# adammoss/nnest

Hardware: AMD Instinct MI355X
Metric: live-point evals/sec (flow-transform + loglike) + log-Z error, x_dim=50 (higher is better)
Workload: dtype f32

## Files before the change

### nnest_amd/csrc/mh_common.h

```cpp
#pragma once
#include "flow_tile.h"
#include "../../include/nnest_hip.h"

namespace nnest {

#ifdef NNEST_STAMP
#define STAMP(v) do { __builtin_amdgcn_sched_barrier(0); v = __builtin_amdgcn_s_memtime(); __builtin_amdgcn_s_waitcnt(0xC07F); __builtin_amdgcn_sched_barrier(0); } while (0)
#else
#define STAMP(v) do { } while (0)
#endif

enum { MH_FORM_AUTO = 0, MH_FORM_IMAGE = 1, MH_FORM_REG = 2, MH_FORM_TEAM = 3, MH_FORM_QUAD = 4, MH_FORM_QUAD1 = 5, MH_FORM_SOLO = 6 };
enum { NNEST_MH_ALL_MOVED = 1 << 30 };
enum { NNEST_MH_WINDOW_VOTES_ONLY = 1 << 28 };
__host__ __device__ inline int mh_flag_lag(int flags) { return (flags >> 8) & 15; }
__host__ __device__ inline int mh_flag_form(int flags) { return (flags >> 16) & 15; }
__host__ __device__ inline int mh_flag_warm(int flags) { return (flags >> 20) & 255; }

enum { MH_SYNC_SHARDS = 8, MH_SYNC_STRIDE = 8 , MH_SYNC_MAX_POLLS = 1 << 20 };
__host__ __device__ inline size_t mh_sync_counter_words(int steps) { return (size_t)(steps + 2) * MH_SYNC_SHARDS * MH_SYNC_STRIDE; }
__host__ __device__ inline size_t mh_sync_window_words(int steps) { return (size_t)((steps + 2) / 32 + 1) * MH_SYNC_SHARDS * MH_SYNC_STRIDE; }
__host__ __device__ inline size_t mh_sync_words(int steps) { return 2 * mh_sync_counter_words(steps) + mh_sync_window_words(steps); }

struct MhArgs {
    const float *img;
    FlowShape s;
    float *z;
    float *x;
    double *logl;
    double loglstar;
    float step_size;
    int steps;
    int C;
    int flags;
    LikeSpec like;
    const float *noise_dz;
    const float *noise_u;
    uint64_t seed;
    uint64_t walker_offset;
    float *hist_x;
    double *hist_logl;
    int *n_accept;
    int *n_call;
    float *scale_out;
    float *x0;
    const float *packed;
    unsigned long long *sync;
    int *sync_err;
};

struct SliceArgs {
    float *z, *x;
    double *logl;
    double loglstar;
    float width;
    int steps, C, max_out, max_shrink;
    LikeSpec like;
    uint64_t seed, walker_offset;
    const float *noise_dz;
    float *hist_x;
    float *x0;
    int *n_call, *n_move, *n_eval;
};

float *mh_first_x_buffer(size_t floats, hipStream_t st);
hipError_t launch_mh_all_moved(const MhArgs &a, hipStream_t st);
hipError_t launch_mh_zero_other_sync(const MhArgs &a, hipStream_t st);

template <int NT>
struct XoshiroNoise {
    Xoshiro128 rn, ru;
    unsigned valid_mask;
    __device__ __forceinline__ void init(uint64_t seed, uint64_t walker, int g, int D) {
        rn = xoshiro_seed(seed, walker, (uint32_t)g, NOISE_STREAM_DZ);
        ru = xoshiro_seed(seed, walker, 0xffffffffu, NOISE_STREAM_U);
        valid_mask = 0;
#pragma unroll
        for (int t = 0; t < NT; ++t)
#pragma unroll
            for (int j = 0; j < 8; ++j)
                if (32 * t + 8 * g + j < D) valid_mask |= 1u << (8 * t + j);
    }
    __device__ __forceinline__ bool relays() const { return false; }
    __device__ __forceinline__ int relayed_total() const { return 0; }
    __device__ __forceinline__ void relay_count(int, int) const {}
    __device__ __forceinline__ void next(float (&nz)[NT][8], float &u) {
#pragma unroll
        for (int t = 0; t < NT; ++t) {
            xoshiro_normal8(rn, nz[t]);
#pragma unroll
            for (int j = 0; j < 8; ++j)
                if (!((valid_mask >> (8 * t + j)) & 1u)) nz[t][j] = 0.f;
        }
        u = xoshiro_uniform(ru);
    }
};

__device__ __forceinline__ void mh_sync_post(unsigned long long *sync, int it, int wg, int accepted) {
    unsigned long long *w = sync + ((size_t)it * MH_SYNC_SHARDS + (wg & (MH_SYNC_SHARDS - 1))) * MH_SYNC_STRIDE;
    __hip_atomic_fetch_add(w, (1ull << 32) | (unsigned long long)(unsigned)accepted, __ATOMIC_RELAXED, __HIP_MEMORY_SCOPE_AGENT);
}
__device__ __forceinline__ unsigned long long mh_sync_read(const unsigned long long *sync, int it) {
    const unsigned long long *w = sync + (size_t)it * MH_SYNC_SHARDS * MH_SYNC_STRIDE;
    unsigned long long s = 0;
#pragma unroll
    for (int k = 0; k < MH_SYNC_SHARDS; ++k)
        s += __hip_atomic_load(w + k * MH_SYNC_STRIDE, __ATOMIC_RELAXED, __HIP_MEMORY_SCOPE_AGENT);
    return s;
}
__device__ __forceinline__ bool mh_sync_failed(const int *err) {
    return err && __hip_atomic_load(err, __ATOMIC_RELAXED, __HIP_MEMORY_SCOPE_AGENT) != 0;
}
__device__ __forceinline__ void mh_sync_fail(int *err, int which = 1) {
    if (err) __hip_atomic_store(err, which, __ATOMIC_RELAXED, __HIP_MEMORY_SCOPE_AGENT);
}
__device__ __forceinline__ int mh_sync_total(const unsigned long long *sync, int it, int nwg, unsigned long long first, int *err) {
    unsigned long long s = first;
    int polls = 0;
    while ((int)(s >> 32) != nwg) {
        if ((polls & 255) == 0 && mh_sync_failed(err)) break;
        if (++polls > MH_SYNC_MAX_POLLS) {
            mh_sync_fail(err);
            break;
        }
        __builtin_amdgcn_s_sleep(2);
        s = mh_sync_read(sync, it);
    }
    return (int)(s & 0xffffffffull);
}

__device__ __forceinline__ void mh_sync_publisher(unsigned long long *sync, int steps, int last_step, int nwg, int nwalkers, int lane, int *err) {
    const int g = lane >> 3, sh = lane & 7;
    unsigned long long *results = sync + mh_sync_counter_words(steps);
    unsigned long long *windows = sync + 2 * mh_sync_counter_words(steps);
    unsigned int wbits = 0;
    int t0 = 1, polls = 0;
    while (t0 <= last_step) {
        const int t = t0 + g;
        const bool live = t <= last_step;
        unsigned long long v = 0;
        if (live) v = __hip_atomic_load(sync + ((size_t)t * MH_SYNC_SHARDS + sh) * MH_SYNC_STRIDE, __ATOMIC_RELAXED, __HIP_MEMORY_SCOPE_AGENT);
        v += __shfl_xor(v, 1);
        v += __shfl_xor(v, 2);
        v += __shfl_xor(v, 4);
        const bool done = live && (int)(v >> 32) == nwg;
        const unsigned long long bal = __ballot(done);
        int ndone = 0;
        while (ndone < 8 && ((bal >> (8 * ndone)) & 1ull)) ++ndone;
        if (g < ndone)
            __hip_atomic_store(results + ((size_t)t * MH_SYNC_SHARDS + sh) * MH_SYNC_STRIDE, (1ull << 63) | (v & 0xffffffffull),
                               __ATOMIC_RELAXED, __HIP_MEMORY_SCOPE_AGENT);
        if (ndone > 0) {
            const unsigned long long up = __ballot(done && 2 * (int)(v & 0xffffffffull) > nwalkers);
            for (int j = 0; j < ndone; ++j) {
                const int s_ = t0 + j, wi = (s_ - 1) >> 5, bi = (s_ - 1) & 31;
                wbits |= (unsigned int)((up >> (8 * j)) & 1ull) << bi;
                if (bi == 31 || j == ndone - 1) {
                    if (lane < MH_SYNC_SHARDS)
                        __hip_atomic_store(windows + ((size_t)wi * MH_SYNC_SHARDS + lane) * MH_SYNC_STRIDE,
                                           ((unsigned long long)(unsigned int)s_ << 32) | wbits, __ATOMIC_RELAXED, __HIP_MEMORY_SCOPE_AGENT);
                    if (bi == 31) wbits = 0;
                }
            }
        }
        t0 += ndone;
        if (ndone == 0) {
            if (++polls > MH_SYNC_MAX_POLLS || ((polls & 255) == 0 && mh_sync_failed(err))) {
                if (polls > MH_SYNC_MAX_POLLS) mh_sync_fail(err, 2);
                for (int tt = t0; tt <= last_step; ++tt)
                    if (lane < MH_SYNC_SHARDS) {
                        __hip_atomic_store(results + ((size_t)tt * MH_SYNC_SHARDS + lane) * MH_SYNC_STRIDE, 1ull << 63, __ATOMIC_RELAXED,
                                           __HIP_MEMORY_SCOPE_AGENT);
                        __hip_atomic_store(windows + ((size_t)((tt - 1) >> 5) * MH_SYNC_SHARDS + lane) * MH_SYNC_STRIDE,
                                           (unsigned long long)(unsigned int)last_step << 32, __ATOMIC_RELAXED, __HIP_MEMORY_SCOPE_AGENT);
                    }
                return;
            }
            __builtin_amdgcn_s_sleep(1);
        }
    }
}
__device__ __forceinline__ unsigned long long mh_result_load(const unsigned long long *sync, int steps, int it, int wg) {
    const unsigned long long *r = sync + mh_sync_counter_words(steps) + ((size_t)it * MH_SYNC_SHARDS + (wg & (MH_SYNC_SHARDS - 1))) * MH_SYNC_STRIDE;
    return __hip_atomic_load(r, __ATOMIC_RELAXED, __HIP_MEMORY_SCOPE_AGENT);
}
__device__ __forceinline__ int mh_result_wait(const unsigned long long *sync, int steps, int it, int wg, unsigned long long first, int *err) {
    unsigned long long v = first;
    int polls = 0;
    while (!(v >> 63)) {
        if ((polls & 255) == 0 && mh_sync_failed(err)) break;
        if (++polls > MH_SYNC_MAX_POLLS) {
            mh_sync_fail(err, 3);
            break;
        }
        __builtin_amdgcn_s_sleep(1);
        v = mh_result_load(sync, steps, it, wg);
    }
    return (int)(v & 0xffffffffull);
}

__device__ __forceinline__ unsigned long long mh_window_load(const unsigned long long *sync, int steps, int it, int wg) {
    const unsigned long long *w = sync + 2 * mh_sync_counter_words(steps) + ((size_t)((it - 1) >> 5) * MH_SYNC_SHARDS + (wg & (MH_SYNC_SHARDS - 1))) * MH_SYNC_STRIDE;
    return __hip_atomic_load(w, __ATOMIC_RELAXED, __HIP_MEMORY_SCOPE_AGENT);
}
__device__ __forceinline__ bool mh_window_vote(const unsigned long long *sync, int steps, int it, int wg, unsigned long long first, int *err) {
    unsigned long long v = first;
    int polls = 0;
    while ((int)(v >> 32) < it) {
        if ((polls & 255) == 0 && mh_sync_failed(err)) break;
        if (++polls > MH_SYNC_MAX_POLLS) {
            mh_sync_fail(err, 4 | (it << 8) | ((wg & 1023) << 20));
            break;
        }
        __builtin_amdgcn_s_sleep(1);
        v = mh_window_load(sync, steps, it, wg);
    }
    return ((v >> ((it - 1) & 31)) & 1ull) != 0;
}

}
```

### nnest_amd/csrc/nnest_solo.hip

```cpp
#include <string.h>
#include <mutex>
#include "mh_common.h"
#include "nnest_internal.h"
#include "solo_loglike.h"
#include "solo_schedule.h"
#include "solo_tile.h"

namespace nnest {

#ifdef NNEST_STAMP
#define PSTAMP(v) do { __builtin_amdgcn_sched_barrier(0); v = __builtin_amdgcn_s_memtime(); __builtin_amdgcn_s_waitcnt(0xC07F); __builtin_amdgcn_sched_barrier(0); } while (0)
#define PSTAMP_DRAINED(v) do { __builtin_amdgcn_sched_barrier(0); __builtin_amdgcn_s_waitcnt(0x0070); v = __builtin_amdgcn_s_memtime(); __builtin_amdgcn_s_waitcnt(0xC07F); __builtin_amdgcn_sched_barrier(0); } while (0)
#ifndef NNEST_STAMP_STEPS
#undef STAMP
#define STAMP(v) do { } while (0)
#endif
#else
#define PSTAMP(v) do { } while (0)
#define PSTAMP_DRAINED(v) do { } while (0)
#endif

static constexpr int SOLO_ETAB = 1024;
__device__ double solo_etab_dev[SOLO_ETAB];
__global__ void solo_etab_kernel() {
    const int k = blockIdx.x * blockDim.x + threadIdx.x;
    if (k < SOLO_ETAB) solo_etab_dev[k] = exp(1.0 / (double)(1 + k));
}
hipError_t solo_prepare_device(int device, hipStream_t st) {
    static std::mutex mu;
    static bool done[64];
    std::lock_guard<std::mutex> g(mu);
    if (device < 0 || device >= 64) return hipErrorInvalidDevice;
    if (done[device]) return hipSuccess;
    hipLaunchKernelGGL(solo_etab_kernel, dim3(SOLO_ETAB / 256), dim3(256), 0, st);
    hipError_t e = hipGetLastError();
    if (e == hipSuccess) e = hipStreamSynchronize(st);
    done[device] = e == hipSuccess;
    return e;
}

template <int U>
__global__ void __launch_bounds__(192) solo_image_kernel(const float *__restrict__ packed, float *__restrict__ limg, int D, int net_params) {
    const int lane = threadIdx.x & 63, b = threadIdx.x >> 6;
    SoloNet<U> nb;
    solo_gather<U>(nb, packed + (size_t)(b * 2 + (lane >= 32 ? 1 : 0)) * net_params, D, (b + 1) & 1, b & 1, lane);
    solo4_store<U>(limg, b, nb, lane);
}
hipError_t launch_solo_image(const float *packed, float *limg, const FlowShape &s, hipStream_t st) {
    if (!s.has_solo_image()) return hipErrorInvalidConfiguration;
    switch (s.NT) {
        case 1: hipLaunchKernelGGL(solo_image_kernel<1>, dim3(1), dim3(192), 0, st, packed, limg, s.D, s.net_params); break;
        case 2: hipLaunchKernelGGL(solo_image_kernel<2>, dim3(1), dim3(192), 0, st, packed, limg, s.D, s.net_params); break;
        case 3: hipLaunchKernelGGL(solo_image_kernel<3>, dim3(1), dim3(192), 0, st, packed, limg, s.D, s.net_params); break;
        case 4: hipLaunchKernelGGL(solo_image_kernel<4>, dim3(1), dim3(192), 0, st, packed, limg, s.D, s.net_params); break;
    }
    return hipGetLastError();
}

template <int U, int WPG> constexpr bool solo_lds_weights() { return U >= 3 || WPG > 4; }
template <int U, int WPG> constexpr int solo_reg_blocks() { return !solo_lds_weights<U, WPG>() ? 3 : (WPG == 4 ? 1 : (U <= 2 && WPG == 8 ? 1 : 0)); }

template <int U>
static __device__ __forceinline__ void solo_pin(float (&v)[2][U]) {
#pragma unroll
    for (int c = 0; c < 2; ++c)
#pragma unroll
        for (int u = 0; u < U; ++u) asm volatile("" : "+v"(v[c][u]));
}

typedef float solo_f32x2 __attribute__((ext_vector_type(2)));
#pragma clang fp contract(off)
static __device__ __forceinline__ double solo_rosenbrock2_paired(const LikeSpec &lk, int D, int lane, const float (&xs)[2][2], float &ld_ride) {
    const int i0 = 4 * (lane & 15);
    const solo_f32x2 sc = {lk.scale, lk.scale};
    const solo_f32x2 P = sc * solo_f32x2{xs[0][0], xs[0][1]};
    const solo_f32x2 Q = sc * solo_f32x2{xs[1][0], xs[1][1]};
    const solo_f32x2 R = {P.y, solo_ror<15>(P.x)};
    const solo_f32x2 aP = P * P, aQ = Q * Q;
    const solo_f32x2 bP = Q - aP, bQ = R - aQ;
    const solo_f32x2 cP = bP * bP, cQ = bQ * bQ;
    const solo_f32x2 eP = 100.0f * cP, eQ = 100.0f * cQ;
    const solo_f32x2 fP = 1.0f - P, fQ = 1.0f - Q;
    const solo_f32x2 qP = fP * fP, qQ = fQ * fQ;
    const solo_f32x2 tP = eP + qP, tQ = eQ + qQ;
    float facc = 0.f;
    facc = facc + ((i0 + 1 < D) ? tP.x : 0.f);
    facc = facc + ((i0 + 2 < D) ? tQ.x : 0.f);
    facc = facc + ((i0 + 3 < D) ? tP.y : 0.f);
    facc = facc + ((i0 + 4 < D) ? tQ.y : 0.f);
    solo_logdet_total_and_row_sum(ld_ride, facc);
    double acc = -(double)facc;
    if (!(fabs(acc) <= 1.79769313486231570e308)) acc = -1e100;
    return acc;
}
#pragma clang fp contract(fast)

enum { MH_SOLO_LAG_INTERNAL = 8 };
template <int U, bool DBG, int LK, int WPG>
__global__ void __launch_bounds__(64 * (WPG + 2)) mh_kernel_solo(MhArgs a) {
    extern __shared__ __attribute__((aligned(16))) float wlds[];
    __shared__ __attribute__((aligned(16))) float nbuf[2][WPG][16][2 * U];
    __shared__ float ubuf[2][WPG];
    __shared__ __attribute__((aligned(16))) uint32_t rawbuf[4 * WPG * 8 * U];
    __shared__ int acc_lds[2][WPG];
    __shared__ float fsbuf[2];
    __shared__ float fs_exact;
    __shared__ float fs_cand[2];
    __shared__ int vote_sel;
    __shared__ double etab[SOLO_ETAB];
    __shared__ __attribute__((aligned(16))) float x0buf[WPG][16][2 * U];

    const int lane = threadIdx.x & 63, wave = __builtin_amdgcn_readfirstlane(threadIdx.x >> 6);
    const int tile = blockIdx.x;
    const int D = a.s.D, S = a.steps, C = a.C;
    const bool recorded = DBG && a.noise_dz;
    const bool dynamic = (a.flags & NNEST_MH_DYNAMIC_BATCH) != 0;
    const bool use_tab = S + 2 <= SOLO_ETAB;
    const bool exact_all = dynamic && mh_flag_lag(a.flags) == 0;
    const bool direct_votes = (a.flags & NNEST_MH_WINDOW_VOTES_ONLY) == 0;
    const int lag = exact_all ? MH_SOLO_LAG_INTERNAL : mh_flag_lag(a.flags);
    const int warm = solo_warm_steps(S, mh_flag_warm(a.flags), dynamic, exact_all);
    constexpr bool LDSW = solo_lds_weights<U, WPG>();
    constexpr int RB = solo_reg_blocks<U, WPG>();
    const int ntiles = (C + WPG - 1) / WPG;
    if (tile >= ntiles) {
        if (dynamic && wave == 0) mh_sync_publisher(a.sync, S, exact_all ? S : max(S - lag, warm), ntiles, C, lane, a.sync_err);
        else if (dynamic && (a.flags & (NNEST_MH_SYNC_ZERO_NEXT | NNEST_MH_SYNC_ZERO_PREV))) {
            const size_t W = (size_t)mh_sync_words(S) + 1;
            unsigned long long *other = (a.flags & NNEST_MH_SYNC_ZERO_NEXT) ? a.sync + W : a.sync - W;
            const int nthr = (int)blockDim.x - 64;
            for (size_t i = threadIdx.x - 64; i < W; i += nthr) other[i] = 0ull;
        }
        return;
    }
    unsigned long long p0 = 0, p1 = 0, p2 = 0, p3 = 0, p4 = 0, p5 = 0, p6 = 0, p7 = 0, p8 = 0;
    (void)p0; (void)p1; (void)p2; (void)p3; (void)p4; (void)p5; (void)p6; (void)p7; (void)p8;
    PSTAMP(p0);
    const float *limg = a.img + a.s.solo_image_offset();
    const int j = wave;
    const int pos = lane & 15;
    const bool translate_half = lane >= 32;
    const bool writer_lane = lane < 16;
    const int row = tile * WPG + j;
    const bool ok = row < C;
    SoloNet<U> net[RB > 0 ? RB : 1];
    float z[2][U];
    double logl = 0.0;
    if (wave < WPG) {
        if constexpr (LDSW) {
            if constexpr (RB == 1) solo_image_load<U>(net[0], limg + (size_t)1 * SOLO4_NF * 64, lane);
        } else {
#pragma unroll
            for (int b = 0; b < 3; ++b) solo_image_load<U>(net[b], limg + (size_t)b * SOLO4_NF * 64, lane);
        }
#pragma unroll
        for (int u = 0; u < U; ++u)
#pragma unroll
            for (int c = 0; c < 2; ++c) {
                const int d = 2 * U * pos + 2 * u + c;
                z[c][u] = (ok && d < D) ? a.z[(size_t)row * D + d] : 0.f;
            }
        logl = ok ? a.logl[row] : 0.0;
    }
    if constexpr (LDSW) solo_image_to_lds<64 * (WPG + 2)>(wlds, limg);
    PSTAMP(p1);
    if (dynamic && use_tab)
        for (int k = threadIdx.x; k < S + 2; k += blockDim.x) etab[k] = solo_etab_dev[k];
    PSTAMP(p2);
    __syncthreads();
    PSTAMP(p3);

    if (wave == WPG) {
        const int g = lane & 3, j = min(lane >> 2, WPG - 1);
        const bool gen = lane < 4 * WPG;
        Xoshiro128 rn = xoshiro_seed(a.seed, a.walker_offset + (uint64_t)(tile * WPG + j), (uint32_t)g, NOISE_STREAM_DZ);
        Xoshiro128 ru = xoshiro_seed(a.seed, a.walker_offset + (uint64_t)(tile * WPG + j), 0xffffffffu, NOISE_STREAM_U);
        constexpr int NQ = 8 * WPG * U;
        unsigned long long n0 = 0, n1 = 0, n2 = 0, n_gen = 0, n_all = 0;
        (void)n0; (void)n1; (void)n2; (void)n_gen; (void)n_all;
        auto draw = [&](int k) {
            if (k > S) return;
            STAMP(n0);
            if (!recorded) {
                if (gen) {
#pragma unroll
                    for (int t = 0; t < 2 * U; ++t) {
                        u32x4 r;
                        r.x = xoshiro_next(rn); r.y = xoshiro_next(rn); r.z = xoshiro_next(rn); r.w = xoshiro_next(rn);
                        *reinterpret_cast<u32x4 *>(&rawbuf[lane * 8 * U + 4 * t]) = r;
                    }
                    const float u = xoshiro_uniform(ru);
                    if (g == 0) ubuf[k & 1][j] = u;
                }
                float *nb = &nbuf[k & 1][0][0][0];
#pragma unroll
                for (int i = 0; i < (NQ + 63) / 64; ++i) {
                    const int q = lane + 64 * i;
                    if (NQ % 64 == 0 || q < NQ) {
                        const u32x4 r = *reinterpret_cast<const u32x4 *>(&rawbuf[4 * q]);
                        const int sl = q / (2 * U), qq = q % (2 * U);
                        const int d0 = 32 * (qq >> 1) + 8 * (sl & 3) + 4 * (qq & 1);
                        float o0, o1, o2, o3;
                        box_muller(r.x, r.y, o0, o1);
                        box_muller(r.z, r.w, o2, o3);
                        const f32x4 o = {d0 < D ? o0 : 0.f, d0 + 1 < D ? o1 : 0.f, d0 + 2 < D ? o2 : 0.f, d0 + 3 < D ? o3 : 0.f};
                        *reinterpret_cast<f32x4 *>(nb + (sl >> 2) * 32 * U + d0) = o;
                    }
                }
            }
            if (!dynamic && lane == 0) fsbuf[k & 1] = a.step_size;
            STAMP(n1);
#ifdef NNEST_STAMP
            n_gen += n1 - n0;
#endif
        };
        STAMP(n2);
        draw(0);
        PSTAMP(p4);
        solo_barrier();
        PSTAMP(p5);
        if (S >= 1) {
            draw(1);
            solo_barrier();
            draw(2);
            for (int k = 1; k <= warm; ++k) {
                solo_barrier();
                solo_barrier();
                draw(k + 2);
                solo_barrier();
            }
            for (int k = solo_first_lagged_fetch(warm); k <= S; ++k) {
                solo_barrier();
                draw(k + 1);
            }
        }
#ifdef NNEST_STAMP
        { unsigned long long n3 = 0; STAMP(n3); n_all = n3 - n2; }
#endif
#ifdef NNEST_STAMP
        PSTAMP(p8);
        if (a.scale_out && lane == 0 && tile == 0) {
            float *o = a.scale_out;
            o[4] = (float)n_gen; o[5] = (float)n_all;
            o[32] = (float)(p1 - p0); o[33] = (float)(p2 - p1); o[34] = (float)(p3 - p2); o[35] = (float)(p4 - p3); o[36] = (float)(p5 - p4);
            o[37] = (float)(p8 - p5); o[38] = (float)(p8 - p0);
        }
#endif
#ifndef NNEST_STAMP
        if (!dynamic && a.scale_out && lane == 0) {
            const int g0 = (tile * WPG + 15) >> 4;
            if (16 * g0 < (tile + 1) * WPG && 16 * g0 < C) a.scale_out[g0] = a.step_size;
        }
#endif
        return;
    }
    if (wave == WPG + 1) {
        if (!dynamic) return;
        double scale = (double)a.step_size;
        int accept = 0, reject = 0;
        const int last = S - lag;
        const unsigned long long *wbase = a.sync + 2 * mh_sync_counter_words(S) + (size_t)(tile & (MH_SYNC_SHARDS - 1)) * MH_SYNC_STRIDE;
#define SOLO_RELAY_ITERATION(k_, q_)                                                                                        \
        {                                                                                                                   \
            const int k = (k_), want = k - lag;                                                                             \
              \
              \
              \
              \
              \
            asm volatile("s_waitcnt vmcnt(2)" : "+v"(q_) : : "memory");                                                     \
            if (want > warm) {                                                                                              \
                const bool up = mh_window_vote(a.sync, S, want, tile, q_, a.sync_err);                                      \
                if (up) accept += 1; else reject += 1;                                                                      \
                if (accept > reject) scale *= use_tab ? etab[accept] : exp(1.0 / (1 + accept));                             \
                if (accept < reject) scale /= use_tab ? etab[reject] : exp(1.0 / (1 + reject));                             \
            }                                                                                                               \
                   \
             \
            if (lane == 0) {                                                                                                \
                const int *ac = acc_lds[k & 1];                                                                             \
                const bool mine = k - 2 > warm;                                 \
                int acs = 0;                                                                                                \
                _Pragma("unroll") for (int w_ = 0; w_ < WPG; ++w_) acs += ac[w_];                                           \
                mh_sync_post(a.sync, mine ? k - 2 : 0, tile, mine ? acs : 0);                                               \
            }                                                                                                               \
            const int ask = min(max(want + 2, 1), max(last, 1));         \
            const unsigned long long *wp = wbase + (size_t)((ask - 1) >> 5) * MH_SYNC_SHARDS * MH_SYNC_STRIDE;              \
            asm volatile("global_load_dwordx2 %0, %1, off sc1" : "=v"(q_) : "v"(wp) : "memory");                            \
              \
            if (lane == 0) fsbuf[k & 1] = (float)scale;                                                                     \
            solo_barrier();                                                                           \
        }
        unsigned long long qa = 0, qb = 0;
        const int k0 = solo_relay_first_iteration(warm);
        if (warm > 0) {
            auto E = [&](int n) { return use_tab ? etab[n] : exp(1.0 / (1 + n)); };
            auto next_scale = [&](int acc, int rej, double sc) {
                if (acc > rej) sc *= E(acc);
                if (acc < rej) sc /= E(rej);
                return sc;
            };
            if (lane == 0) {
                fsbuf[0] = (float)scale;
                fs_cand[0] = (float)next_scale(accept + 1, reject, scale);
                fs_cand[1] = (float)next_scale(accept, reject + 1, scale);
            }
            solo_barrier();
            if (lane == 0) fsbuf[1] = (float)scale;
            solo_barrier();
            for (int k = 1; k <= warm; ++k) {
                solo_barrier();
                if (lane == 0) {
                    const int *ac = acc_lds[k & 1];
                    int acs = 0;
#pragma unroll
                    for (int w_ = 0; w_ < WPG; ++w_) acs += ac[w_];
                    mh_sync_post(a.sync, k, tile, acs);
                    fsbuf[(k + 1) & 1] = (float)scale;
                }
                solo_barrier();
                const bool up = direct_votes ? 2 * mh_sync_total(a.sync, k, ntiles, 0ull, a.sync_err) > C
                                             : mh_window_vote(a.sync, S, k, tile, 0ull, a.sync_err);
                if (up) accept += 1; else reject += 1;
                scale = next_scale(accept, reject, scale);
                if (lane == 0) {
                    vote_sel = up ? 0 : 1;
                    fs_exact = (float)scale;
                    fs_cand[0] = (float)next_scale(accept + 1, reject, scale);
                    fs_cand[1] = (float)next_scale(accept, reject + 1, scale);
                }
                solo_barrier();
            }
        }
        for (int k2 = k0; k2 <= S; k2 += 2) {
            SOLO_RELAY_ITERATION(k2, qa)
            if (k2 + 1 <= S) SOLO_RELAY_ITERATION(k2 + 1, qb)
        }
#undef SOLO_RELAY_ITERATION
        asm volatile("s_waitcnt vmcnt(0)" : "+v"(qa), "+v"(qb) : : "memory");
        if (exact_all) {
            solo_barrier();
            if (lane == 0) {
                const int *ac = acc_lds[S & 1];
                int acs = 0;
#pragma unroll
                for (int w_ = 0; w_ < WPG; ++w_) acs += ac[w_];
                mh_sync_post(a.sync, S, tile, acs);
            }
            const bool up = direct_votes ? 2 * mh_sync_total(a.sync, S, ntiles, 0ull, a.sync_err) > C : mh_window_vote(a.sync, S, S, tile, 0ull, a.sync_err);
            if (up) accept += 1; else reject += 1;
            if (accept > reject) scale *= use_tab ? etab[accept] : exp(1.0 / (1 + accept));
            if (accept < reject) scale /= use_tab ? etab[reject] : exp(1.0 / (1 + reject));
        }
#ifndef NNEST_STAMP
        if (a.scale_out && lane == 0) {
            const int g0 = (tile * WPG + 15) >> 4;
            if (16 * g0 < (tile + 1) * WPG && 16 * g0 < C) a.scale_out[g0] = (float)scale;
        }
#endif
        return;
    }

    const LikeSpec like = a.like;
    const double loglstar = a.loglstar;
    const bool free_mode = (a.flags & NNEST_MH_UNCONSTRAINED) != 0;
    PSTAMP(p4);
    const unsigned sel = translate_half ? 0xffffffffu : 0u;
    const bool h1 = (lane & 16) != 0;
    auto inverse = [&](float (&xs)[2][U]) {
        if constexpr (LDSW) {
            float ld = solo_coupling_inverse4<U>(Solo4Lds{wlds + (size_t)2 * SOLO4_NF * 64, lane}, sel, h1, xs[1], xs[0]);
            if constexpr (RB == 1) ld += solo_coupling_inverse4<U>(Solo4Reg<U>{net[0]}, sel, h1, xs[0], xs[1]);
            else ld += solo_coupling_inverse4<U>(Solo4Lds{wlds + (size_t)1 * SOLO4_NF * 64, lane}, sel, h1, xs[0], xs[1]);
            ld += solo_coupling_inverse4<U>(Solo4Lds{wlds, lane}, sel, h1, xs[1], xs[0]);
            return ld;
        } else {
            float ld;
            solo_coupling_inverse<U, true>(net[2], sel, h1, xs[1], xs[0], ld);
            solo_coupling_inverse<U, false>(net[1], sel, h1, xs[0], xs[1], ld);
            solo_coupling_inverse<U, false>(net[0], sel, h1, xs[1], xs[0], ld);
            return ld;
        }
    };

    constexpr bool X_LATE = !DBG && !LDSW;
    float x[2][U];
#pragma unroll
    for (int u = 0; u < U; ++u)
#pragma unroll
        for (int c = 0; c < 2; ++c) x[c][u] = z[c][u];
    float ld = solo_logdet_total(inverse(x));
    int n_acc = 0, n_call = 0;

    auto store_row = [&](float *base, size_t r, const float (&v)[2][U]) {
#pragma unroll
        for (int u = 0; u < U; ++u)
#pragma unroll
            for (int c = 0; c < 2; ++c) {
                const int d = 2 * U * pos + 2 * u + c;
                if (d < D) base[r * D + d] = v[c][u];
            }
    };
    if (writer_lane && a.x) {
#pragma unroll
        for (int u = 0; u < U; ++u)
#pragma unroll
            for (int c = 0; c < 2; ++c) x0buf[j][pos][2 * u + c] = x[c][u];
    }
    if (DBG && writer_lane && ok) {
        if (a.hist_x) store_row(a.hist_x, (size_t)row * (S + 1), x);
        if (a.hist_logl && pos == 0) a.hist_logl[(size_t)row * (S + 1)] = logl;
    }

    float nz[2 * U], u_next = 0.f, fs_next = a.step_size;
    auto read_noise = [&](int par) {
        if (!recorded) {
#pragma unroll
            for (int k = 0; k < 2 * U; ++k) nz[k] = nbuf[par][j][pos][k];
            u_next = ubuf[par][j];
        }
        fs_next = fsbuf[par];
    };
    auto fetch_noise = [&](int par, auto &...zp) {
        solo_barrier();
        (solo_pin(zp), ...);
        read_noise(par);
    };
    constexpr bool LATE_FETCH = LK == NNEST_LIKE_ROSENBROCK && U == 2 && !DBG && !LDSW;
    PSTAMP(p5);
    fetch_noise(0);
    PSTAMP(p6);

    unsigned long long st0 = 0, st1 = 0, st2 = 0, st3 = 0, a_prop = 0, a_inv = 0, a_post = 0, a_tot = 0;
    (void)st0; (void)st1; (void)st2; (void)st3; (void)a_prop; (void)a_inv; (void)a_post; (void)a_tot;
    struct Prop { float zp[2][U], xp[2][U]; float ldp; double lp; bool pre, acc; };
    auto propose = [&](int it, float fs, float (&zp)[2][U], float &u) {
        if (recorded) {
#pragma unroll
            for (int uu = 0; uu < U; ++uu)
#pragma unroll
                for (int c = 0; c < 2; ++c) {
                    const int d = 2 * U * pos + 2 * uu + c;
                    const float dz = (ok && d < D) ? a.noise_dz[((size_t)(it - 1) * C + row) * D + d] : 0.f;
                    zp[c][uu] = __builtin_fmaf(dz, fs, z[c][uu]);
                }
            u = ok ? a.noise_u[(size_t)(it - 1) * C + row] : 1.f;
        } else {
#pragma unroll
            for (int uu = 0; uu < U; ++uu) {
                zp[0][uu] = __builtin_fmaf(nz[2 * uu], fs, z[0][uu]);
                zp[1][uu] = __builtin_fmaf(nz[2 * uu + 1], fs, z[1][uu]);
            }
            u = u_next;
        }
    };
    auto finish = [&](Prop &r, float u, int late_par = -1) {
#pragma unroll
        for (int c = 0; c < 2; ++c)
#pragma unroll
            for (int uu = 0; uu < U; ++uu) r.xp[c][uu] = r.zp[c][uu];
        STAMP(st1);
        constexpr bool RIDE = LK == NNEST_LIKE_ROSENBROCK;
        r.ldp = RIDE ? inverse(r.xp) : solo_logdet_total(inverse(r.xp));
        if (late_par >= 0) {
            asm volatile("" : "+v"(r.ldp) : : "memory");
            read_noise(late_par);
        }
        STAMP(st2);
        if constexpr (RIDE && U == 2 && !DBG && !LDSW) r.lp = solo_rosenbrock2_paired(like, D, lane, r.xp, r.ldp);
        else if constexpr (RIDE) r.lp = solo_loglike<U, LK>(like, D, lane, r.xp, &r.ldp);
        int okl = 1;
#pragma unroll
        for (int c = 0; c < 2; ++c)
#pragma unroll
            for (int uu = 0; uu < U; ++uu) okl &= !(r.xp[c][uu] < -1.f || r.xp[c][uu] > 1.f);
        const bool inb = __ballot(okl != 0) == ~0ull;
        float log_ratio = inb ? (r.ldp - ld) : -INFINITY;
        float ratio = fminf(__expf(log_ratio), 1.0f);
        if (log_ratio != log_ratio) ratio = log_ratio;
        r.pre = ok && (u < ratio);
        if constexpr (!RIDE) r.lp = solo_loglike<U, LK>(like, D, lane, r.xp);
        r.acc = r.pre && (r.lp > loglstar);
        if (free_mode) {
            const double lr = inb ? (double)(r.ldp - ld) + (r.lp - logl) : -INFINITY;
            const double rt = fmin(exp(lr), 1.0);
            r.acc = ok && ((double)u < rt);
        }
    };
    auto apply = [&](int it, int par, const Prop &r) {
        n_call += (free_mode ? ok : r.pre) ? 1 : 0;
        n_acc += r.acc ? 1 : 0;
#pragma unroll
        for (int c = 0; c < 2; ++c)
#pragma unroll
            for (int uu = 0; uu < U; ++uu) {
                z[c][uu] = r.acc ? r.zp[c][uu] : z[c][uu];
                if constexpr (!X_LATE) x[c][uu] = r.acc ? r.xp[c][uu] : x[c][uu];
            }
        ld = r.acc ? r.ldp : ld;
        logl = r.acc ? r.lp : logl;
        if (dynamic && lane == 0) acc_lds[par][j] = r.acc ? 1 : 0;
        if (DBG && writer_lane && ok) {
            if (a.hist_x) store_row(a.hist_x, (size_t)row * (S + 1) + it, x);
            if (a.hist_logl && pos == 0) a.hist_logl[(size_t)row * (S + 1) + it] = logl;
        }
    };
    if (warm > 0) {
        Prop cur;
        {
            float u;
            propose(1, fs_next, cur.zp, u);
            fetch_noise(1, cur.zp);
            finish(cur, u);
        }
        for (int it = 1; it <= warm; ++it) {
            STAMP(st0);
            apply(it, it & 1, cur);
            solo_barrier();
            const float f0 = fs_cand[0], f1 = fs_cand[1];
            Prop c1;
            float u;
            propose(it + 1, f0, cur.zp, u);
            propose(it + 1, f1, c1.zp, u);
            fetch_noise((it + 1) & 1, cur.zp, c1.zp);
            finish(cur, u);
            finish(c1, u);
            solo_barrier();
            if (vote_sel != 0) cur = c1;
            fs_next = fs_exact;
            STAMP(st3);
#ifdef NNEST_STAMP
            a_prop += st1 - st0; a_inv += st2 - st1; a_post += st3 - st2; a_tot += st3 - st0;
#endif
        }
        apply(warm + 1, (warm + 1) & 1, cur);
    }
    auto straight_step = [&](int it, int par) {
        STAMP(st0);
        Prop r;
        float u;
        propose(it, fs_next, r.zp, u);
        if constexpr (LATE_FETCH) {
            solo_barrier();
            solo_pin(r.zp);
            finish(r, u, par);
        } else {
            fetch_noise(par, r.zp);
            finish(r, u);
        }
        apply(it, par, r);
        STAMP(st3);
#ifdef NNEST_STAMP
        a_prop += st1 - st0; a_inv += st2 - st1; a_post += st3 - st2; a_tot += st3 - st0;
#endif
    };
    {
        int it = solo_first_straight_step(warm);
        if (it <= S && (it & 1)) { straight_step(it, 1); ++it; }
        for (; it < S; it += 2) {
            straight_step(it, 0);
            straight_step(it + 1, 1);
        }
        if (it <= S) straight_step(it, 0);
    }
    if (exact_all) solo_barrier();
    PSTAMP(p7);
#ifdef NNEST_STAMP
    if (a.scale_out && lane == 0 && tile == 0) {
        float *o = a.scale_out;
        if (j == 0) { o[0] = (float)a_tot; o[1] = (float)a_prop; o[2] = (float)a_inv; o[3] = (float)a_post; }
        if (j < 4) { o[8 + 2 * j] = (float)a_inv; o[9 + 2 * j] = (float)a_post; }
    }
#endif
    bool all_moved = n_acc > 0;
    if (a.x) {
        if constexpr (X_LATE) {
#pragma unroll
            for (int u = 0; u < U; ++u)
#pragma unroll
                for (int c = 0; c < 2; ++c) x[c][u] = z[c][u];
            (void)inverse(x);
        }
        bool mine = true;
        if (writer_lane) {
#pragma unroll
            for (int u = 0; u < U; ++u)
#pragma unroll
                for (int c = 0; c < 2; ++c) {
                    const int d = 2 * U * pos + 2 * u + c;
                    const float x0 = x0buf[j][pos][2 * u + c];
                    mine = mine && (d >= D || x[c][u] != x0);
                }
        }
        all_moved = (__ballot(mine) & 0xffffull) == 0xffffull;
    }
    if (writer_lane && ok) {
        store_row(a.z, (size_t)row, z);
        if (a.x) store_row(a.x, (size_t)row, x);
        if (pos == 0) {
            a.logl[row] = logl;
            if (a.n_accept) a.n_accept[row] = n_acc | (all_moved ? NNEST_MH_ALL_MOVED : 0);
            if (a.n_call) a.n_call[row] = n_call;
        }
    }
#ifdef NNEST_STAMP
    PSTAMP_DRAINED(p8);
    if (a.scale_out && lane == 0 && tile == 0 && j == 0) {
        float *o = a.scale_out;
        o[16] = (float)(p1 - p0); o[17] = (float)(p2 - p1); o[18] = (float)(p3 - p2); o[19] = (float)(p4 - p3); o[20] = (float)(p5 - p4);
        o[21] = (float)(p6 - p5); o[22] = (float)(p7 - p6); o[23] = (float)(p8 - p7); o[24] = (float)(p8 - p0);
    }
#endif
}

template <int U>
static __device__ __forceinline__ void slice_normals(uint64_t seed, uint64_t walker, uint32_t step, int pos, int D, float (&e)[2][U]) {
    const int d0 = 2 * U * pos;
    f32x4 q[(2 * U + 3) / 4 + 1];
    const int q0 = d0 >> 2;
#pragma unroll
    for (int k = 0; k < (2 * U + 3) / 4 + 1; ++k) q[k] = noise_normal4(seed, walker, step, (uint32_t)(q0 + k), NOISE_STREAM_DZ);
#pragma unroll
    for (int u = 0; u < U; ++u)
#pragma unroll
        for (int c = 0; c < 2; ++c) {
            const int d = d0 + 2 * u + c, k = (d >> 2) - q0, r = d & 3;
            float v = 0.f;
#pragma unroll
            for (int kk = 0; kk < (2 * U + 3) / 4 + 1; ++kk)
                if (kk == k) v = r == 0 ? q[kk].x : (r == 1 ? q[kk].y : (r == 2 ? q[kk].z : q[kk].w));
            e[c][u] = d < D ? v : 0.f;
        }
}

template <int U, int LK>
__global__ void __launch_bounds__(256) slice_kernel_solo(SliceArgs a, FlowShape s, const float *limg) {
    extern __shared__ __attribute__((aligned(16))) float wlds[];
    __shared__ __attribute__((aligned(16))) float x0buf[4][16][2 * U];
    const int lane = threadIdx.x & 63, wave = __builtin_amdgcn_readfirstlane(threadIdx.x >> 6);
    const int D = s.D, S = a.steps, C = a.C;
    constexpr bool LDSW = solo_lds_weights<U, 4>();
    if constexpr (LDSW) {
        solo_image_to_lds<256>(wlds, limg);
        __syncthreads();
    }
    const int pos = lane & 15;
    const bool translate_half = lane >= 32, writer_lane = lane < 16;
    const int row = blockIdx.x * 4 + wave;
    const bool ok = row < C;
    if (!ok) return;
    const LikeSpec like = a.like;
    const double loglstar = a.loglstar;
    SoloNet<U> net[LDSW ? 1 : 3];
    if constexpr (!LDSW) {
#pragma unroll
        for (int b = 0; b < 3; ++b) solo_image_load<U>(net[b], limg + (size_t)b * SOLO4_NF * 64, lane);
    }
    const unsigned sel = translate_half ? 0xffffffffu : 0u;
    const bool h1 = (lane & 16) != 0;
    auto inverse = [&](float (&xs)[2][U]) {
        if constexpr (LDSW) {
            float ld = solo_coupling_inverse4<U>(Solo4Lds{wlds + (size_t)2 * SOLO4_NF * 64, lane}, sel, h1, xs[1], xs[0]);
            ld += solo_coupling_inverse4<U>(Solo4Lds{wlds + (size_t)1 * SOLO4_NF * 64, lane}, sel, h1, xs[0], xs[1]);
            ld += solo_coupling_inverse4<U>(Solo4Lds{wlds, lane}, sel, h1, xs[1], xs[0]);
            return ld;
        } else {
            float ld;
            solo_coupling_inverse<U, true>(net[2], sel, h1, xs[1], xs[0], ld);
            solo_coupling_inverse<U, false>(net[1], sel, h1, xs[0], xs[1], ld);
            solo_coupling_inverse<U, false>(net[0], sel, h1, xs[1], xs[0], ld);
            return ld;
        }
    };
    auto store_row = [&](float *base, size_t r, const float (&v)[2][U]) {
#pragma unroll
        for (int u = 0; u < U; ++u)
#pragma unroll
            for (int c = 0; c < 2; ++c) {
                const int d = 2 * U * pos + 2 * u + c;
                if (d < D) base[r * D + d] = v[c][u];
            }
    };
    float z[2][U], x[2][U];
#pragma unroll
    for (int u = 0; u < U; ++u)
#pragma unroll
        for (int c = 0; c < 2; ++c) {
            const int d = 2 * U * pos + 2 * u + c;
            z[c][u] = d < D ? a.z[(size_t)row * D + d] : 0.f;
            x[c][u] = z[c][u];
        }
    float ld = solo_logdet_total(inverse(x));
    double logl = a.logl[row];
    if (writer_lane && a.x) {
#pragma unroll
        for (int u = 0; u < U; ++u)
#pragma unroll
            for (int c = 0; c < 2; ++c) x0buf[wave][pos][2 * u + c] = x[c][u];
    }
    if (writer_lane && a.hist_x) store_row(a.hist_x, (size_t)row * (S + 1), x);
    const uint64_t walker = a.walker_offset + (uint64_t)row;
    int n_call = 0, n_move = 0, n_eval = 0;
    float zc[2][U], xc[2][U], ldc = 0.f;
    double lc = 0.0;
    for (int it = 1; it <= S; ++it) {
        float e[2][U];
        if (a.noise_dz) {
#pragma unroll
            for (int u = 0; u < U; ++u)
#pragma unroll
                for (int c = 0; c < 2; ++c) {
                    const int d = 2 * U * pos + 2 * u + c;
                    e[c][u] = d < D ? a.noise_dz[((size_t)(it - 1) * C + row) * D + d] : 0.f;
                }
        } else {
            slice_normals<U>(a.seed, walker, (uint32_t)it, pos, D, e);
        }
        const float u0 = noise_uniform(a.seed, walker, 64u * (uint32_t)it + 0u), u1 = noise_uniform(a.seed, walker, 64u * (uint32_t)it + 1u);
        const float logy = ld + __logf(u1);
        auto inside = [&](float t) -> bool {
            const float tw = t * a.width;
#pragma unroll
            for (int u = 0; u < U; ++u)
#pragma unroll
                for (int c = 0; c < 2; ++c) { zc[c][u] = __builtin_fmaf(e[c][u], tw, z[c][u]); xc[c][u] = zc[c][u]; }
            ldc = solo_logdet_total(inverse(xc));
            int okl = 1;
#pragma unroll
            for (int c = 0; c < 2; ++c)
#pragma unroll
                for (int u = 0; u < U; ++u) okl &= !(xc[c][u] < -1.f || xc[c][u] > 1.f);
            const bool inb = __ballot(okl != 0) == ~0ull;
            const bool pre = inb && (ldc > logy);
            lc = solo_loglike<U, LK>(like, D, lane, xc);
            n_eval += 1;
            n_call += pre ? 1 : 0;
            return pre && (lc > loglstar);
        };
        float tl = -u0, tr = 1.0f - u0;
        if (a.max_out > 0) {
            const int B = 2 * a.max_out;
            int n = 0;
            while (n <= B && inside(tl)) { tl -= 1.0f; n += 1; }
            while (n <= B && inside(tr)) { tr += 1.0f; n += 1; }
            if (n > B) {
                tl = -u0;
                tr = 1.0f - u0;
                const int nl = slice_stepout_left(a.seed, walker, (uint32_t)it, a.max_out);
                for (int j = 0; j < nl; ++j) { if (!inside(tl)) break; tl -= 1.0f; }
                for (int j = 0; j < B - nl; ++j) { if (!inside(tr)) break; tr += 1.0f; }
            }
        }
        bool moved = false;
        for (int k = 0; k < a.max_shrink; ++k) {
            const float uk = noise_uniform(a.seed, walker, 64u * (uint32_t)it + 2u + (uint32_t)k);
            const float t = __builtin_fmaf(tr - tl, uk, tl);
            if (inside(t)) { moved = true; break; }
            if (t < 0.f) tl = t; else tr = t;
        }
        if (moved) {
#pragma unroll
            for (int c = 0; c < 2; ++c)
#pragma unroll
                for (int u = 0; u < U; ++u) { z[c][u] = zc[c][u]; x[c][u] = xc[c][u]; }
            ld = ldc; logl = lc; n_move += 1;
        }
        if (writer_lane && a.hist_x) store_row(a.hist_x, (size_t)row * (S + 1) + it, x);
    }
    bool all_moved = n_move > 0;
    if (a.x) {
        bool mine = true;
        if (writer_lane) {
#pragma unroll
            for (int u = 0; u < U; ++u)
#pragma unroll
                for (int c = 0; c < 2; ++c) {
                    const int d = 2 * U * pos + 2 * u + c;
                    const float x0 = x0buf[wave][pos][2 * u + c];
                    mine = mine && (d >= D || x[c][u] != x0);
                }
        }
        all_moved = (__ballot(mine) & 0xffffull) == 0xffffull;
    }
    if (writer_lane) {
        store_row(a.z, (size_t)row, z);
        if (a.x) store_row(a.x, (size_t)row, x);
        if (pos == 0) {
            a.logl[row] = logl;
            if (a.n_call) a.n_call[row] = n_call;
            if (a.n_move) a.n_move[row] = n_move | (all_moved ? NNEST_MH_ALL_MOVED : 0);
            if (a.n_eval) a.n_eval[row] = n_eval;
        }
    }
}

__global__ void slice_fill_noise_kernel(float *__restrict__ dz, int steps, int C, int D, uint64_t seed, uint64_t walker_offset) {
    const long nq = (long)steps * C * ((D + 3) / 4);
    for (long i = (long)blockIdx.x * blockDim.x + threadIdx.x; i < nq; i += (long)gridDim.x * blockDim.x) {
        const int Q = (D + 3) / 4, q = (int)(i % Q), c = (int)((i / Q) % C), it = (int)(i / ((long)Q * C)) + 1;
        const f32x4 n = noise_normal4(seed, walker_offset + (uint64_t)c, (uint32_t)it, (uint32_t)q, NOISE_STREAM_DZ);
        float *o = dz + ((size_t)(it - 1) * C + c) * D + 4 * q;
        if (4 * q + 0 < D) o[0] = n.x;
        if (4 * q + 1 < D) o[1] = n.y;
        if (4 * q + 2 < D) o[2] = n.z;
        if (4 * q + 3 < D) o[3] = n.w;
    }
}

template <int U, int LK>
static hipError_t launch_slice_k(const FlowShape &s, const float *limg, const SliceArgs &a, hipStream_t st) {
    const size_t lds = solo_lds_weights<U, 4>() ? (size_t)3 * SOLO4_NF * 64 * sizeof(float) : 0;
    hipError_t e = hipFuncSetAttribute(reinterpret_cast<const void *>(slice_kernel_solo<U, LK>), hipFuncAttributeMaxDynamicSharedMemorySize, (int)lds);
    if (e != hipSuccess) return e;
    hipLaunchKernelGGL((slice_kernel_solo<U, LK>), dim3((a.C + 3) / 4), dim3(256), lds, st, a, s, limg);
    return hipGetLastError();
}

bool slice_form_eligible(const FlowShape &s) {
    return s.kind == FLOW_KIND_NVP && s.H == 16 && s.B == 3 && s.L == 1 && s.scale_mode == 0 && s.NT >= 1 && s.NT <= 4;
}

hipError_t launch_slice_solo(const FlowShape &s, const float *limg, const SliceArgs &a, hipStream_t st) {
    if (a.C <= 0) return hipSuccess;
    if (!slice_form_eligible(s)) return hipErrorInvalidConfiguration;
    const bool rosen = a.like.id == NNEST_LIKE_ROSENBROCK;
    switch (s.NT) {
        case 1: return rosen ? launch_slice_k<1, NNEST_LIKE_ROSENBROCK>(s, limg, a, st) : launch_slice_k<1, -1>(s, limg, a, st);
        case 2: return rosen ? launch_slice_k<2, NNEST_LIKE_ROSENBROCK>(s, limg, a, st) : launch_slice_k<2, -1>(s, limg, a, st);
        case 3: return rosen ? launch_slice_k<3, NNEST_LIKE_ROSENBROCK>(s, limg, a, st) : launch_slice_k<3, -1>(s, limg, a, st);
        case 4: return rosen ? launch_slice_k<4, NNEST_LIKE_ROSENBROCK>(s, limg, a, st) : launch_slice_k<4, -1>(s, limg, a, st);
    }
    return hipErrorInvalidConfiguration;
}

hipError_t launch_slice_fill_noise(float *dz, int steps, int C, int D, uint64_t seed, uint64_t walker_offset, hipStream_t st) {
    hipLaunchKernelGGL(slice_fill_noise_kernel, dim3(256), dim3(256), 0, st, dz, steps, C, D, seed, walker_offset);
    return hipGetLastError();
}

int solo_walkers_per_group(int C, int num_cu) {
    static const int pinned = [] { const char *e = getenv("NNEST_SOLO_WPG"); return e ? atoi(e) : 0; }();
    for (int wpg = 4; wpg <= 12; wpg += 4) {
        if (pinned && wpg != pinned) continue;
        if ((C + wpg - 1) / wpg + 1 <= num_cu) return wpg;
    }
    return 0;
}

bool solo_form_eligible(const MhArgs &a, int num_cu) {
    const FlowShape &s = a.s;
    if (s.H != 16 || s.B != 3 || s.L != 1 || s.scale_mode != 0 || s.NT < 1 || s.NT > 4) return false;
    if (a.flags & NNEST_MH_DYNAMIC_STEP) return false;
    if ((a.flags & NNEST_MH_DYNAMIC_BATCH) && (mh_flag_lag(a.flags) == 1 || mh_flag_lag(a.flags) == 2)) return false;
    const int wpg = solo_walkers_per_group(a.C, num_cu);
    if (wpg != 4 && (a.noise_dz || a.hist_x || a.hist_logl)) return false;
    return wpg != 0;
}

template <int U, bool DBG, int LK, int WPG>
static hipError_t launch_solo_k(const MhArgs &a, hipStream_t st) {
    const int batch = (a.flags & NNEST_MH_DYNAMIC_BATCH) ? 1 : 0;
    const int grid = (a.C + WPG - 1) / WPG + batch;
    const size_t lds = solo_lds_weights<U, WPG>() ? (size_t)3 * SOLO4_NF * 64 * sizeof(float) : 0;
    hipError_t e = hipFuncSetAttribute(reinterpret_cast<const void *>(mh_kernel_solo<U, DBG, LK, WPG>),
                                       hipFuncAttributeMaxDynamicSharedMemorySize, (int)lds);
    if (e != hipSuccess) return e;
    hipLaunchKernelGGL((mh_kernel_solo<U, DBG, LK, WPG>), dim3(grid), dim3(64 * (WPG + 2)), lds, st, a);
    return hipGetLastError();
}
template <int U, bool DBG, int LK>
static hipError_t launch_solo_w(const MhArgs &a, int wpg, hipStream_t st) {
    if (wpg == 4) return launch_solo_k<U, DBG, LK, 4>(a, st);
    if constexpr (!DBG) {
        if (wpg == 8) return launch_solo_k<U, DBG, LK, 8>(a, st);
        if (wpg == 12) return launch_solo_k<U, DBG, LK, 12>(a, st);
    }
    return hipErrorInvalidConfiguration;
}

hipError_t launch_mh_solo(const MhArgs &a_in, int num_cu, hipStream_t st) {
    MhArgs a = a_in;
    static const bool window_votes = [] { const char *e = getenv("NNEST_SOLO_VOTE"); return e && !strcmp(e, "window"); }();
    if (window_votes) a.flags |= NNEST_MH_WINDOW_VOTES_ONLY;
    const bool dbg = a.noise_dz || a.hist_x || a.hist_logl;
    const int wpg = solo_walkers_per_group(a.C, num_cu);
    if (!dbg && a.like.id == NNEST_LIKE_ROSENBROCK) {
        if (a.s.NT == 1) return launch_solo_w<1, false, NNEST_LIKE_ROSENBROCK>(a, wpg, st);
        if (a.s.NT == 2) return launch_solo_w<2, false, NNEST_LIKE_ROSENBROCK>(a, wpg, st);
        if (a.s.NT == 3) return launch_solo_w<3, false, NNEST_LIKE_ROSENBROCK>(a, wpg, st);
        if (a.s.NT == 4) return launch_solo_w<4, false, NNEST_LIKE_ROSENBROCK>(a, wpg, st);
    }
    switch (a.s.NT) {
        case 1: return dbg ? launch_solo_w<1, true, -1>(a, wpg, st) : launch_solo_w<1, false, -1>(a, wpg, st);
        case 2: return dbg ? launch_solo_w<2, true, -1>(a, wpg, st) : launch_solo_w<2, false, -1>(a, wpg, st);
        case 3: return dbg ? launch_solo_w<3, true, -1>(a, wpg, st) : launch_solo_w<3, false, -1>(a, wpg, st);
        case 4: return dbg ? launch_solo_w<4, true, -1>(a, wpg, st) : launch_solo_w<4, false, -1>(a, wpg, st);
    }
    return hipErrorInvalidConfiguration;
}

}
```

Measured before the change: 1.052 billion.

## Post warmup votes early per tile and poll both vote outcomes speculatively

During warmup, each walker wave adds its accept bits for both candidate scales into a workgroup-shared counter as soon as its proposals finish. The last wave to arrive posts a packed word with up/down counts to the global sync buffer, instead of waiting for a barrier and having lane 0 sum the LDS array. The coordinating wave precomputes both candidate next-scale values and issues vote reads with asm global loads, using a DPP shard reduction and a fast path when the first read already shows all tiles. This shortens the cross-workgroup vote critical path. The cost is limiting C to 65535 walkers and adding inline asm fragility.

```diff
diff --git a/nnest_amd/csrc/mh_common.h b/nnest_amd/csrc/mh_common.h
--- a/nnest_amd/csrc/mh_common.h
+++ b/nnest_amd/csrc/mh_common.h
@@ -96,9 +96,12 @@
     }
 };
 
+__device__ __forceinline__ void mh_sync_post_word(unsigned long long *sync, int it, int wg, unsigned long long word) {
+    unsigned long long *w = sync + ((size_t)it * MH_SYNC_SHARDS + (wg & (MH_SYNC_SHARDS - 1))) * MH_SYNC_STRIDE;
+    __hip_atomic_fetch_add(w, word, __ATOMIC_RELAXED, __HIP_MEMORY_SCOPE_AGENT);
+}
 __device__ __forceinline__ void mh_sync_post(unsigned long long *sync, int it, int wg, int accepted) {
-    unsigned long long *w = sync + ((size_t)it * MH_SYNC_SHARDS + (wg & (MH_SYNC_SHARDS - 1))) * MH_SYNC_STRIDE;
-    __hip_atomic_fetch_add(w, (1ull << 32) | (unsigned long long)(unsigned)accepted, __ATOMIC_RELAXED, __HIP_MEMORY_SCOPE_AGENT);
+    mh_sync_post_word(sync, it, wg, (1ull << 32) | (unsigned long long)(unsigned)accepted);
 }
 __device__ __forceinline__ unsigned long long mh_sync_read(const unsigned long long *sync, int it) {
     const unsigned long long *w = sync + (size_t)it * MH_SYNC_SHARDS * MH_SYNC_STRIDE;
@@ -114,7 +117,7 @@
 __device__ __forceinline__ void mh_sync_fail(int *err, int which = 1) {
     if (err) __hip_atomic_store(err, which, __ATOMIC_RELAXED, __HIP_MEMORY_SCOPE_AGENT);
 }
-__device__ __forceinline__ int mh_sync_total(const unsigned long long *sync, int it, int nwg, unsigned long long first, int *err) {
+__device__ __forceinline__ unsigned long long mh_sync_total_word(const unsigned long long *sync, int it, int nwg, unsigned long long first, int *err) {
     unsigned long long s = first;
     int polls = 0;
     while ((int)(s >> 32) != nwg) {
@@ -126,7 +129,10 @@
         __builtin_amdgcn_s_sleep(2);
         s = mh_sync_read(sync, it);
     }
-    return (int)(s & 0xffffffffull);
+    return s;
+}
+__device__ __forceinline__ int mh_sync_total(const unsigned long long *sync, int it, int nwg, unsigned long long first, int *err) {
+    return (int)(mh_sync_total_word(sync, it, nwg, first, err) & 0xffffffffull);
 }
 
 __device__ __forceinline__ void mh_sync_publisher(unsigned long long *sync, int steps, int last_step, int nwg, int nwalkers, int lane, int *err) {
diff --git a/nnest_amd/csrc/nnest_solo.hip b/nnest_amd/csrc/nnest_solo.hip
--- a/nnest_amd/csrc/nnest_solo.hip
+++ b/nnest_amd/csrc/nnest_solo.hip
@@ -5,6 +5,7 @@
 #include "solo_loglike.h"
 #include "solo_schedule.h"
 #include "solo_tile.h"
+#include "solo_votes.h"
 
 namespace nnest {
 
@@ -14,10 +15,15 @@
 #ifndef NNEST_STAMP_STEPS
 #undef STAMP
 #define STAMP(v) do { } while (0)
+#define STAMP_DRAINED(v) do { } while (0)
+#else
+#define STAMP_DRAINED(v) PSTAMP_DRAINED(v)
+#define SOLO_STAMP_VOTES 1
 #endif
 #else
 #define PSTAMP(v) do { } while (0)
 #define PSTAMP_DRAINED(v) do { } while (0)
+#define STAMP_DRAINED(v) do { } while (0)
 #endif
 
 static constexpr int SOLO_ETAB = 1024;
@@ -95,6 +101,17 @@
 }
 #pragma clang fp contract(fast)
 
+static __device__ __forceinline__ unsigned solo_sum8(unsigned v) {
+    v += (unsigned)__builtin_amdgcn_update_dpp(0, (int)v, 0xB1, 0xf, 0xf, true);
+    v += (unsigned)__builtin_amdgcn_update_dpp(0, (int)v, 0x4E, 0xf, 0xf, true);
+    v += (unsigned)__builtin_amdgcn_update_dpp(0, (int)v, 0x141, 0xf, 0xf, true);
+    return v;
+}
+static __device__ __forceinline__ unsigned long long solo_shard_sum(unsigned long long q) {
+    const unsigned lo = solo_sum8((unsigned)q), hi = solo_sum8((unsigned)(q >> 32));
+    return ((unsigned long long)(unsigned)__builtin_amdgcn_readfirstlane((int)hi) << 32) | (unsigned long long)(unsigned)__builtin_amdgcn_readfirstlane((int)lo);
+}
+
 enum { MH_SOLO_LAG_INTERNAL = 8 };
 template <int U, bool DBG, int LK, int WPG>
 __global__ void __launch_bounds__(64 * (WPG + 2)) mh_kernel_solo(MhArgs a) {
@@ -107,6 +124,8 @@
     __shared__ float fs_exact;
     __shared__ float fs_cand[2];
     __shared__ int vote_sel;
+    __shared__ unsigned tile_votes;
+    static_assert(WPG <= SOLO_VOTES_MAX_TILE, "the tile's word counts its waves in 8-bit fields");
     __shared__ double etab[SOLO_ETAB];
     __shared__ __attribute__((aligned(16))) float x0buf[WPG][16][2 * U];
 
@@ -166,6 +185,7 @@
     PSTAMP(p1);
     if (dynamic && use_tab)
         for (int k = threadIdx.x; k < S + 2; k += blockDim.x) etab[k] = solo_etab_dev[k];
+    if (threadIdx.x == 0) tile_votes = 0u;
     PSTAMP(p2);
     __syncthreads();
     PSTAMP(p3);
@@ -300,6 +320,11 @@
                 if (acc < rej) sc /= E(rej);
                 return sc;
             };
+            unsigned long long v_a = 0, v_q0 = 0, v_q1 = 0, v_first = 0, v_known = 0, v_b = 0;
+            unsigned long long vs_q0 = 0, vs_q1 = 0, vs_first = 0, vs_known = 0, vs_b = 0;
+            int vn_votes = 0, vn_polls = 0, vh1 = 0, vh2 = 0, vh3 = 0, vh4 = 0;
+            (void)v_a; (void)v_q0; (void)v_q1; (void)v_first; (void)v_known; (void)v_b; (void)vs_q0; (void)vs_q1; (void)vs_first; (void)vs_known; (void)vs_b;
+            (void)vn_votes; (void)vn_polls; (void)vh1; (void)vh2; (void)vh3; (void)vh4;
             if (lane == 0) {
                 fsbuf[0] = (float)scale;
                 fs_cand[0] = (float)next_scale(accept + 1, reject, scale);
@@ -308,29 +333,100 @@
             solo_barrier();
             if (lane == 0) fsbuf[1] = (float)scale;
             solo_barrier();
+            bool prev_up = true;
+            unsigned long long qv0 = 0, qv1 = 0;
+            const unsigned long long *vbase = a.sync + (size_t)(lane & (MH_SYNC_SHARDS - 1)) * MH_SYNC_STRIDE;
+#define SOLO_VOTE_REQUEST(q_, k_) asm volatile("global_load_dwordx2 %0, %1, off sc1" : "=v"(q_) : "v"(vbase + (size_t)(k_) * MH_SYNC_SHARDS * MH_SYNC_STRIDE) : "memory")
+#define SOLO_VOTE_LANDED(n_) asm volatile("s_waitcnt vmcnt(" #n_ ")" : "+v"(qv0), "+v"(qv1) : : "memory")
+            STAMP(v_b);
             for (int k = 1; k <= warm; ++k) {
+                SOLO_VOTE_LANDED(0);
                 solo_barrier();
+                STAMP(v_a);
                 if (lane == 0) {
-                    const int *ac = acc_lds[k & 1];
-                    int acs = 0;
-#pragma unroll
-                    for (int w_ = 0; w_ < WPG; ++w_) acs += ac[w_];
-                    mh_sync_post(a.sync, k, tile, acs);
+                    if (!direct_votes) {
+                        const int *ac = acc_lds[k & 1];
+                        int acs = 0;
+#pragma unroll
+                        for (int w_ = 0; w_ < WPG; ++w_) acs += ac[w_];
+                        mh_sync_post(a.sync, k, tile, acs);
+                    }
                     fsbuf[(k + 1) & 1] = (float)scale;
                 }
                 solo_barrier();
-                const bool up = direct_votes ? 2 * mh_sync_total(a.sync, k, ntiles, 0ull, a.sync_err) > C
-                                             : mh_window_vote(a.sync, S, k, tile, 0ull, a.sync_err);
+                const double s_up = next_scale(accept + 1, reject, scale), s_dn = next_scale(accept, reject + 1, scale);
+                const float c_uu = (float)next_scale(accept + 2, reject, s_up), c_ud = (float)next_scale(accept + 1, reject + 1, s_up);
+                STAMP(v_q0);
+                if (direct_votes) {
+                    asm volatile("" : : "v"(c_uu), "v"(c_ud) : "memory");
+                    SOLO_VOTE_REQUEST(qv0, k);
+                }
+                const float c_du = (float)next_scale(accept + 1, reject + 1, s_dn), c_dd = (float)next_scale(accept, reject + 2, s_dn);
+                bool up;
+                if (direct_votes) {
+                    asm volatile("" : : "v"(c_du), "v"(c_dd) : "memory");
+                    STAMP(v_q1);
+                    SOLO_VOTE_REQUEST(qv1, k);
+                    SOLO_VOTE_LANDED(1);
+                    STAMP(v_first);
+                    unsigned long long word = solo_shard_sum(qv0);
+                    int polls = 1;
+                    if (solo_votes_tiles(word) != ntiles) {
+                        SOLO_VOTE_LANDED(0);
+                        word = solo_shard_sum(qv1);
+                        polls = 2;
+                        int misses = 0;
+                        while (solo_votes_tiles(word) != ntiles) {
+                            if (++misses > MH_SYNC_MAX_POLLS) {
+                                mh_sync_fail(a.sync_err);
+                                break;
+                            }
+                            __builtin_amdgcn_s_sleep(2);
+                            SOLO_VOTE_REQUEST(qv0, k);
+                            const bool failed = (misses & 255) == 1 && mh_sync_failed(a.sync_err);
+                            SOLO_VOTE_LANDED(0);
+                            word = solo_shard_sum(qv0);
+                            polls += 1;
+                            if (failed) break;
+                        }
+                    }
+                    (void)polls;
+#ifdef SOLO_STAMP_VOTES
+                    vn_polls += polls; vh1 += polls == 1; vh2 += polls == 2; vh3 += polls == 3; vh4 += polls >= 4;
+#endif
+                    up = solo_votes_up(word, prev_up, C);
+                } else {
+                    up = mh_window_vote(a.sync, S, k, tile, 0ull, a.sync_err);
+                }
+                prev_up = up;
+                STAMP(v_known);
+#ifdef SOLO_STAMP_VOTES
+                vs_q0 += v_q0 - v_b; vs_q1 += v_q1 - v_q0; vs_first += v_first - v_q0; vs_known += v_known - v_q0;
+#endif
                 if (up) accept += 1; else reject += 1;
-                scale = next_scale(accept, reject, scale);
+                scale = up ? s_up : s_dn;
                 if (lane == 0) {
                     vote_sel = up ? 0 : 1;
                     fs_exact = (float)scale;
-                    fs_cand[0] = (float)next_scale(accept + 1, reject, scale);
-                    fs_cand[1] = (float)next_scale(accept, reject + 1, scale);
+                    fs_cand[0] = up ? c_uu : c_du;
+                    fs_cand[1] = up ? c_ud : c_dd;
                 }
                 solo_barrier();
-            }
+                STAMP(v_b);
+#ifdef SOLO_STAMP_VOTES
+                vs_b += v_b - v_known; vn_votes += 1;
+#endif
+            }
+            SOLO_VOTE_LANDED(0);
+#undef SOLO_VOTE_REQUEST
+#undef SOLO_VOTE_LANDED
+#ifdef SOLO_STAMP_VOTES
+            if (a.scale_out && lane == 0 && tile == 0) {
+                float *o = a.scale_out;
+                o[40] = (float)vn_votes; o[41] = (float)vs_q0; o[42] = (float)vs_q1; o[43] = (float)vs_first; o[44] = (float)vn_polls;
+                o[45] = (float)vs_known; o[46] = (float)vh1; o[47] = (float)vh2; o[48] = (float)vh3; o[49] = (float)vh4; o[54] = (float)vs_b;
+            }
+#endif
         }
         for (int k2 = k0; k2 <= S; k2 += 2) {
             SOLO_RELAY_ITERATION(k2, qa)
@@ -433,6 +529,8 @@
 
     unsigned long long st0 = 0, st1 = 0, st2 = 0, st3 = 0, a_prop = 0, a_inv = 0, a_post = 0, a_tot = 0;
     (void)st0; (void)st1; (void)st2; (void)st3; (void)a_prop; (void)a_inv; (void)a_post; (void)a_tot;
+    unsigned long long sb0 = 0, sb1 = 0, a_bwait = 0;
+    (void)sb0; (void)sb1; (void)a_bwait;
     struct Prop { float zp[2][U], xp[2][U]; float ldp; double lp; bool pre, acc; };
     auto propose = [&](int it, float fs, float (&zp)[2][U], float &u) {
         if (recorded) {
@@ -506,12 +604,24 @@
         }
     };
     if (warm > 0) {
+        const bool early_votes = direct_votes;
+        auto post_early = [&](int step, bool acc_up, bool acc_down) {
+            if (early_votes && lane == 0) {
+                const unsigned add = solo_votes_tile_add(acc_up, acc_down);
+                const unsigned old = __hip_atomic_fetch_add(&tile_votes, add, __ATOMIC_RELAXED, __HIP_MEMORY_SCOPE_WORKGROUP);
+                if (solo_votes_tile_arrived(old) == WPG - 1) {
+                    __hip_atomic_store(&tile_votes, 0u, __ATOMIC_RELAXED, __HIP_MEMORY_SCOPE_WORKGROUP);
+                    mh_sync_post_word(a.sync, step, tile, solo_votes_tile_post(old + add));
+                }
+            }
+        };
         Prop cur;
         {
             float u;
             propose(1, fs_next, cur.zp, u);
             fetch_noise(1, cur.zp);
             finish(cur, u);
+            post_early(1, cur.acc, cur.acc);
         }
         for (int it = 1; it <= warm; ++it) {
             STAMP(st0);
@@ -525,7 +635,13 @@
             fetch_noise((it + 1) & 1, cur.zp, c1.zp);
             finish(cur, u);
             finish(c1, u);
+            if (it < warm) post_early(it + 1, cur.acc, c1.acc);
+            STAMP(sb0);
             solo_barrier();
+            STAMP(sb1);
+#ifdef SOLO_STAMP_VOTES
+            a_bwait += sb1 - sb0;
+#endif
             if (vote_sel != 0) cur = c1;
             fs_next = fs_exact;
             STAMP(st3);
@@ -570,6 +686,7 @@
         float *o = a.scale_out;
         if (j == 0) { o[0] = (float)a_tot; o[1] = (float)a_prop; o[2] = (float)a_inv; o[3] = (float)a_post; }
         if (j < 4) { o[8 + 2 * j] = (float)a_inv; o[9 + 2 * j] = (float)a_post; }
+        if (j < 4) o[50 + j] = (float)a_bwait;
     }
 #endif
     bool all_moved = n_acc > 0;
@@ -840,6 +957,7 @@
 
 int solo_walkers_per_group(int C, int num_cu) {
     static const int pinned = [] { const char *e = getenv("NNEST_SOLO_WPG"); return e ? atoi(e) : 0; }();
+    if (C > SOLO_VOTES_MAX_WALKERS) return 0;
     for (int wpg = 4; wpg <= 12; wpg += 4) {
         if (pinned && wpg != pinned) continue;
         if ((C + wpg - 1) / wpg + 1 <= num_cu) return wpg;
diff --git a/nnest_amd/csrc/solo_votes.h b/nnest_amd/csrc/solo_votes.h
--- /dev/null
+++ b/nnest_amd/csrc/solo_votes.h
@@ -0,0 +1,31 @@
+#pragma once
+
+#if defined(__HIPCC__) || defined(__CUDACC__)
+#define SOLO_VOTES_FN __host__ __device__ constexpr
+#else
+#define SOLO_VOTES_FN constexpr
+#endif
+
+namespace nnest {
+
+enum { SOLO_VOTES_FIELD_BITS = 16, SOLO_VOTES_MAX_WALKERS = (1 << SOLO_VOTES_FIELD_BITS) - 1 };
+
+SOLO_VOTES_FN unsigned long long solo_votes_pack(unsigned up, unsigned down) {
+    return (1ull << 32) | ((unsigned long long)(down & 0xffffu) << SOLO_VOTES_FIELD_BITS) | (unsigned long long)(up & 0xffffu);
+}
+SOLO_VOTES_FN int solo_votes_tiles(unsigned long long word) { return (int)(word >> 32); }
+SOLO_VOTES_FN int solo_votes_accepted(unsigned long long word, bool prev_up) {
+    return (int)((prev_up ? word : word >> SOLO_VOTES_FIELD_BITS) & 0xffffull);
+}
+SOLO_VOTES_FN bool solo_votes_up(unsigned long long word, bool prev_up, int walkers) { return 2 * solo_votes_accepted(word, prev_up) > walkers; }
+
+enum { SOLO_VOTES_TILE_BITS = 8, SOLO_VOTES_MAX_TILE = (1 << SOLO_VOTES_TILE_BITS) - 1 };
+SOLO_VOTES_FN unsigned solo_votes_tile_add(bool acc_up, bool acc_down) {
+    return (1u << (2 * SOLO_VOTES_TILE_BITS)) | ((acc_down ? 1u : 0u) << SOLO_VOTES_TILE_BITS) | (acc_up ? 1u : 0u);
+}
+SOLO_VOTES_FN int solo_votes_tile_arrived(unsigned w) { return (int)(w >> (2 * SOLO_VOTES_TILE_BITS)); }
+SOLO_VOTES_FN unsigned long long solo_votes_tile_post(unsigned w) {
+    return solo_votes_pack(w & (unsigned)SOLO_VOTES_MAX_TILE, (w >> SOLO_VOTES_TILE_BITS) & (unsigned)SOLO_VOTES_MAX_TILE);
+}
+
+}
diff --git a/profiles/r11/k4_solo_loop.s b/profiles/r11/k4_solo_loop.s
--- /dev/null
+++ b/profiles/r11/k4_solo_loop.s
@@ -0,0 +1,790 @@
+	v_mov_b32_e32 v192, s51
+	ds_write_b32 v192, v191 offset:16
+	s_or_b64 exec, exec, s[12:13]
+	v_and_b32_e32 v142, 0xffff, v142
+	v_and_b32_e32 v1, 0xffff, v1
+	s_add_i32 s19, s19, 2
+	v_add3_u32 v166, v166, v142, v1
+	v_add3_u32 v167, v167, v185, v191
+	v_cndmask_b32_e64 v29, v29, v188, s[14:15]
+	v_cndmask_b32_e64 v93, v93, v189, s[14:15]
+	v_cndmask_b32_e64 v143, v143, v187, s[14:15]
+	v_cndmask_b32_e64 v145, v145, v165, s[14:15]
+	v_cndmask_b32_e64 v144, v144, v164, s[14:15]
+	v_cndmask_b32_e64 v177, v177, v190, s[14:15]
+	s_cmp_lt_i32 s19, s37
+	v_cndmask_b32_e64 v89, v89, v186, s[14:15]
+	s_cbranch_scc0 1198
+	s_waitcnt lgkmcnt(0)
+	v_fma_f32 v187, v138, v169, v29
+	v_fma_f32 v186, v139, v169, v143
+	v_fma_f32 v188, v140, v169, v93
+	v_fma_f32 v169, v141, v169, v89
+	s_waitcnt lgkmcnt(0)
+	s_barrier
+	s_nop 0
+	v_mov_b32_e32 v1, v186
+	v_mov_b32_e32 v138, v169
+	v_bfi_b32 v141, v171, v188, v187
+	v_mov_b32_dpp v1, v186 row_ror:8 row_mask:0xa bank_mask:0xf
+	v_mov_b32_dpp v138, v169 row_ror:8 row_mask:0xa bank_mask:0xf
+	v_fma_f32 v139, v1, v94, v90
+	v_mul_f32_e32 v140, v138, v102
+	v_fmac_f32_dpp v140, v138, v103 row_ror:1 row_mask:0xf bank_mask:0xf
+	v_fmac_f32_dpp v139, v1, v95 row_ror:1 row_mask:0xf bank_mask:0xf
+	v_fmac_f32_dpp v140, v138, v104 row_ror:2 row_mask:0xf bank_mask:0xf
+	v_fmac_f32_dpp v139, v1, v96 row_ror:2 row_mask:0xf bank_mask:0xf
+	v_fmac_f32_dpp v140, v138, v105 row_ror:3 row_mask:0xf bank_mask:0xf
+	v_fmac_f32_dpp v139, v1, v97 row_ror:3 row_mask:0xf bank_mask:0xf
+	v_fmac_f32_dpp v140, v138, v106 row_ror:4 row_mask:0xf bank_mask:0xf
+	v_fmac_f32_dpp v139, v1, v98 row_ror:4 row_mask:0xf bank_mask:0xf
+	v_fmac_f32_dpp v140, v138, v107 row_ror:5 row_mask:0xf bank_mask:0xf
+	v_fmac_f32_dpp v139, v1, v99 row_ror:5 row_mask:0xf bank_mask:0xf
+	v_fmac_f32_dpp v140, v138, v108 row_ror:6 row_mask:0xf bank_mask:0xf
+	v_fmac_f32_dpp v139, v1, v100 row_ror:6 row_mask:0xf bank_mask:0xf
+	v_fmac_f32_dpp v140, v138, v109 row_ror:7 row_mask:0xf bank_mask:0xf
+	v_fmac_f32_dpp v139, v1, v101 row_ror:7 row_mask:0xf bank_mask:0xf
+	v_add_f32_e32 v138, v139, v140
+	v_mov_b32_dpp v1, v140 row_ror:8 row_mask:0xf bank_mask:0xf
+	v_add_f32_dpp v1, v139, v1 row_ror:8 row_mask:0xf bank_mask:0xf
+	s_nop 1
+	v_permlane16_swap_b32_e32 v138, v1
+	v_add_f32_e32 v139, v138, v1
+	v_exp_f32_e32 v1, v139
+	v_max_f32_e32 v138, 0, v139
+	v_add_f32_e32 v1, 1.0, v1
+	v_rcp_f32_e32 v1, v1
+	s_nop 0
+	v_fma_f32 v1, v1, -2.0, 1.0
+	v_bfi_b32 v139, v170, v138, v1
+	v_fma_f32 v1, v139, v110, v91
+	s_nop 0
+	v_mul_f32_dpp v138, v139, v111 row_ror:1 row_mask:0xf bank_mask:0xf
+	v_fmac_f32_dpp v1, v139, v112 row_ror:2 row_mask:0xf bank_mask:0xf
+	v_fmac_f32_dpp v138, v139, v113 row_ror:3 row_mask:0xf bank_mask:0xf
+	v_fmac_f32_dpp v1, v139, v114 row_ror:4 row_mask:0xf bank_mask:0xf
+	v_fmac_f32_dpp v138, v139, v115 row_ror:5 row_mask:0xf bank_mask:0xf
+	v_fmac_f32_dpp v1, v139, v116 row_ror:6 row_mask:0xf bank_mask:0xf
+	v_fmac_f32_dpp v138, v139, v117 row_ror:7 row_mask:0xf bank_mask:0xf
+	v_add_f32_e32 v139, v1, v138
+	v_add_f32_e32 v140, v1, v138
+	s_nop 1
+	v_permlane16_swap_b32_e32 v139, v140
+	v_add_f32_e32 v139, v139, v140
+	v_exp_f32_e32 v1, v139
+	v_max_f32_e32 v138, 0, v139
+	v_add_f32_e32 v1, 1.0, v1
+	v_rcp_f32_e32 v1, v1
+	s_nop 0
+	v_fma_f32 v1, v1, -2.0, 1.0
+	v_bfi_b32 v139, v170, v138, v1
+	v_fma_f32 v1, v139, v118, v92
+	v_mov_b32_e32 v138, 0
+	v_fmac_f32_dpp v138, v139, v122 row_ror:8 row_mask:0xf bank_mask:0xf
+	v_fmac_f32_dpp v1, v139, v119 row_ror:1 row_mask:0xf bank_mask:0xf
+	v_fmac_f32_dpp v138, v139, v123 row_ror:9 row_mask:0xf bank_mask:0xf
+	v_fmac_f32_dpp v1, v139, v120 row_ror:2 row_mask:0xf bank_mask:0xf
+	v_fmac_f32_dpp v138, v139, v124 row_ror:10 row_mask:0xf bank_mask:0xf
+	v_fmac_f32_dpp v1, v139, v121 row_ror:3 row_mask:0xf bank_mask:0xf
+	v_fmac_f32_dpp v138, v139, v125 row_ror:11 row_mask:0xf bank_mask:0xf
+	v_fmac_f32_dpp v1, v139, v126 row_ror:4 row_mask:0xf bank_mask:0xf
+	v_fmac_f32_dpp v138, v139, v130 row_ror:12 row_mask:0xf bank_mask:0xf
+	v_fmac_f32_dpp v1, v139, v127 row_ror:5 row_mask:0xf bank_mask:0xf
+	v_fmac_f32_dpp v138, v139, v131 row_ror:13 row_mask:0xf bank_mask:0xf
+	v_fmac_f32_dpp v1, v139, v128 row_ror:6 row_mask:0xf bank_mask:0xf
+	v_fmac_f32_dpp v138, v139, v132 row_ror:14 row_mask:0xf bank_mask:0xf
+	v_fmac_f32_dpp v1, v139, v129 row_ror:7 row_mask:0xf bank_mask:0xf
+	v_fmac_f32_dpp v138, v139, v133 row_ror:15 row_mask:0xf bank_mask:0xf
+	v_add_f32_e32 v139, v1, v138
+	v_add_f32_e32 v140, v1, v138
+	s_nop 1
+	v_permlane32_swap_b32_e32 v139, v140
+	v_mul_f32_e32 v1, 0xbfb8aa3b, v139
+	v_exp_f32_e32 v1, v1
+	v_sub_f32_e32 v138, v141, v140
+	v_mul_f32_e32 v142, v138, v1
+	v_mul_f32_e32 v185, v138, v1
+	v_mul_f32_e32 v189, -1.0, v139
+	s_nop 0
+	v_permlane16_swap_b32_e32 v142, v185
+	s_nop 0
+	v_mov_b32_e32 v1, v142
+	v_mov_b32_e32 v138, v185
+	v_bfi_b32 v141, v171, v169, v186
+	v_mov_b32_dpp v1, v142 row_ror:8 row_mask:0xa bank_mask:0xf
+	v_mov_b32_dpp v138, v185 row_ror:8 row_mask:0xa bank_mask:0xf
+	v_fma_f32 v139, v1, v50, v86
+	v_mul_f32_e32 v140, v138, v34
+	v_fmac_f32_dpp v140, v138, v35 row_ror:1 row_mask:0xf bank_mask:0xf
+	v_fmac_f32_dpp v139, v1, v51 row_ror:1 row_mask:0xf bank_mask:0xf
+	v_fmac_f32_dpp v140, v138, v36 row_ror:2 row_mask:0xf bank_mask:0xf
+	v_fmac_f32_dpp v139, v1, v52 row_ror:2 row_mask:0xf bank_mask:0xf
+	v_fmac_f32_dpp v140, v138, v37 row_ror:3 row_mask:0xf bank_mask:0xf
+	v_fmac_f32_dpp v139, v1, v53 row_ror:3 row_mask:0xf bank_mask:0xf
+	v_fmac_f32_dpp v140, v138, v58 row_ror:4 row_mask:0xf bank_mask:0xf
+	v_fmac_f32_dpp v139, v1, v54 row_ror:4 row_mask:0xf bank_mask:0xf
+	v_fmac_f32_dpp v140, v138, v59 row_ror:5 row_mask:0xf bank_mask:0xf
+	v_fmac_f32_dpp v139, v1, v55 row_ror:5 row_mask:0xf bank_mask:0xf
+	v_fmac_f32_dpp v140, v138, v60 row_ror:6 row_mask:0xf bank_mask:0xf
+	v_fmac_f32_dpp v139, v1, v56 row_ror:6 row_mask:0xf bank_mask:0xf
+	v_fmac_f32_dpp v140, v138, v61 row_ror:7 row_mask:0xf bank_mask:0xf
+	v_fmac_f32_dpp v139, v1, v57 row_ror:7 row_mask:0xf bank_mask:0xf
+	v_add_f32_e32 v138, v139, v140
+	v_mov_b32_dpp v1, v140 row_ror:8 row_mask:0xf bank_mask:0xf
+	v_add_f32_dpp v1, v139, v1 row_ror:8 row_mask:0xf bank_mask:0xf
+	s_nop 1
+	v_permlane16_swap_b32_e32 v138, v1
+	v_add_f32_e32 v139, v138, v1
+	v_exp_f32_e32 v1, v139
+	v_max_f32_e32 v138, 0, v139
+	v_add_f32_e32 v1, 1.0, v1
+	v_rcp_f32_e32 v1, v1
+	s_nop 0
+	v_fma_f32 v1, v1, -2.0, 1.0
+	v_bfi_b32 v139, v170, v138, v1
+	v_fma_f32 v1, v139, v62, v87
+	s_nop 0
+	v_mul_f32_dpp v138, v139, v63 row_ror:1 row_mask:0xf bank_mask:0xf
+	v_fmac_f32_dpp v1, v139, v64 row_ror:2 row_mask:0xf bank_mask:0xf
+	v_fmac_f32_dpp v138, v139, v65 row_ror:3 row_mask:0xf bank_mask:0xf
+	v_fmac_f32_dpp v1, v139, v66 row_ror:4 row_mask:0xf bank_mask:0xf
+	v_fmac_f32_dpp v138, v139, v67 row_ror:5 row_mask:0xf bank_mask:0xf
+	v_fmac_f32_dpp v1, v139, v68 row_ror:6 row_mask:0xf bank_mask:0xf
+	v_fmac_f32_dpp v138, v139, v69 row_ror:7 row_mask:0xf bank_mask:0xf
+	v_add_f32_e32 v139, v1, v138
+	v_add_f32_e32 v140, v1, v138
+	s_nop 1
+	v_permlane16_swap_b32_e32 v139, v140
+	v_add_f32_e32 v139, v139, v140
+	v_exp_f32_e32 v1, v139
+	v_max_f32_e32 v138, 0, v139
+	v_add_f32_e32 v1, 1.0, v1
+	v_rcp_f32_e32 v1, v1
+	s_nop 0
+	v_fma_f32 v1, v1, -2.0, 1.0
+	v_bfi_b32 v139, v170, v138, v1
+	v_fma_f32 v1, v139, v70, v88
+	v_mov_b32_e32 v138, 0
+	v_fmac_f32_dpp v138, v139, v78 row_ror:8 row_mask:0xf bank_mask:0xf
+	v_fmac_f32_dpp v1, v139, v71 row_ror:1 row_mask:0xf bank_mask:0xf
+	v_fmac_f32_dpp v138, v139, v79 row_ror:9 row_mask:0xf bank_mask:0xf
+	v_fmac_f32_dpp v1, v139, v72 row_ror:2 row_mask:0xf bank_mask:0xf
+	v_fmac_f32_dpp v138, v139, v80 row_ror:10 row_mask:0xf bank_mask:0xf
+	v_fmac_f32_dpp v1, v139, v73 row_ror:3 row_mask:0xf bank_mask:0xf
+	v_fmac_f32_dpp v138, v139, v81 row_ror:11 row_mask:0xf bank_mask:0xf
+	v_fmac_f32_dpp v1, v139, v74 row_ror:4 row_mask:0xf bank_mask:0xf
+	v_fmac_f32_dpp v138, v139, v82 row_ror:12 row_mask:0xf bank_mask:0xf
+	v_fmac_f32_dpp v1, v139, v75 row_ror:5 row_mask:0xf bank_mask:0xf
+	v_fmac_f32_dpp v138, v139, v83 row_ror:13 row_mask:0xf bank_mask:0xf
+	v_fmac_f32_dpp v1, v139, v76 row_ror:6 row_mask:0xf bank_mask:0xf
+	v_fmac_f32_dpp v138, v139, v84 row_ror:14 row_mask:0xf bank_mask:0xf
+	v_fmac_f32_dpp v1, v139, v77 row_ror:7 row_mask:0xf bank_mask:0xf
+	v_fmac_f32_dpp v138, v139, v85 row_ror:15 row_mask:0xf bank_mask:0xf
+	v_add_f32_e32 v139, v1, v138
+	v_add_f32_e32 v140, v1, v138
+	s_nop 1
+	v_permlane32_swap_b32_e32 v139, v140
+	v_mul_f32_e32 v1, 0xbfb8aa3b, v139
+	v_exp_f32_e32 v1, v1
+	v_sub_f32_e32 v138, v141, v140
+	v_mul_f32_e32 v164, v138, v1
+	v_mul_f32_e32 v165, v138, v1
+	v_sub_f32_e32 v189, v189, v139
+	s_nop 0
+	v_permlane16_swap_b32_e32 v164, v165
+	s_nop 0
+	v_mov_b32_e32 v1, v164
+	v_mov_b32_e32 v138, v165
+	v_bfi_b32 v141, v171, v185, v142
+	v_mov_b32_dpp v1, v164 row_ror:8 row_mask:0xa bank_mask:0xf
+	v_mov_b32_dpp v138, v165 row_ror:8 row_mask:0xa bank_mask:0xf
+	v_fma_f32 v139, v1, v30, v26
+	v_mul_f32_e32 v140, v138, v42
+	v_fmac_f32_dpp v140, v138, v43 row_ror:1 row_mask:0xf bank_mask:0xf
+	v_fmac_f32_dpp v139, v1, v31 row_ror:1 row_mask:0xf bank_mask:0xf
+	v_fmac_f32_dpp v140, v138, v44 row_ror:2 row_mask:0xf bank_mask:0xf
+	v_fmac_f32_dpp v139, v1, v32 row_ror:2 row_mask:0xf bank_mask:0xf
+	v_fmac_f32_dpp v140, v138, v45 row_ror:3 row_mask:0xf bank_mask:0xf
+	v_fmac_f32_dpp v139, v1, v33 row_ror:3 row_mask:0xf bank_mask:0xf
+	v_fmac_f32_dpp v140, v138, v46 row_ror:4 row_mask:0xf bank_mask:0xf
+	v_fmac_f32_dpp v139, v1, v38 row_ror:4 row_mask:0xf bank_mask:0xf
+	v_fmac_f32_dpp v140, v138, v47 row_ror:5 row_mask:0xf bank_mask:0xf
+	v_fmac_f32_dpp v139, v1, v39 row_ror:5 row_mask:0xf bank_mask:0xf
+	v_fmac_f32_dpp v140, v138, v48 row_ror:6 row_mask:0xf bank_mask:0xf
+	v_fmac_f32_dpp v139, v1, v40 row_ror:6 row_mask:0xf bank_mask:0xf
+	v_fmac_f32_dpp v140, v138, v49 row_ror:7 row_mask:0xf bank_mask:0xf
+	v_fmac_f32_dpp v139, v1, v41 row_ror:7 row_mask:0xf bank_mask:0xf
+	v_add_f32_e32 v138, v139, v140
+	v_mov_b32_dpp v1, v140 row_ror:8 row_mask:0xf bank_mask:0xf
+	v_add_f32_dpp v1, v139, v1 row_ror:8 row_mask:0xf bank_mask:0xf
+	s_nop 1
+	v_permlane16_swap_b32_e32 v138, v1
+	v_add_f32_e32 v139, v138, v1
+	v_exp_f32_e32 v1, v139
+	v_max_f32_e32 v138, 0, v139
+	v_add_f32_e32 v1, 1.0, v1
+	v_rcp_f32_e32 v1, v1
+	s_nop 0
+	v_fma_f32 v1, v1, -2.0, 1.0
+	v_bfi_b32 v139, v170, v138, v1
+	v_fma_f32 v1, v139, v6, v27
+	s_nop 0
+	v_mul_f32_dpp v138, v139, v7 row_ror:1 row_mask:0xf bank_mask:0xf
+	v_fmac_f32_dpp v1, v139, v8 row_ror:2 row_mask:0xf bank_mask:0xf
+	v_fmac_f32_dpp v138, v139, v9 row_ror:3 row_mask:0xf bank_mask:0xf
+	v_fmac_f32_dpp v1, v139, v14 row_ror:4 row_mask:0xf bank_mask:0xf
+	v_fmac_f32_dpp v138, v139, v15 row_ror:5 row_mask:0xf bank_mask:0xf
+	v_fmac_f32_dpp v1, v139, v16 row_ror:6 row_mask:0xf bank_mask:0xf
+	v_fmac_f32_dpp v138, v139, v17 row_ror:7 row_mask:0xf bank_mask:0xf
+	v_add_f32_e32 v139, v1, v138
+	v_add_f32_e32 v140, v1, v138
+	s_nop 1
+	v_permlane16_swap_b32_e32 v139, v140
+	v_add_f32_e32 v139, v139, v140
+	v_exp_f32_e32 v1, v139
+	v_max_f32_e32 v138, 0, v139
+	v_add_f32_e32 v1, 1.0, v1
+	v_rcp_f32_e32 v1, v1
+	s_nop 0
+	v_fma_f32 v1, v1, -2.0, 1.0
+	v_bfi_b32 v139, v170, v138, v1
+	v_fma_f32 v1, v139, v2, v28
+	v_mov_b32_e32 v138, 0
+	v_fmac_f32_dpp v138, v139, v18 row_ror:8 row_mask:0xf bank_mask:0xf
+	v_fmac_f32_dpp v1, v139, v3 row_ror:1 row_mask:0xf bank_mask:0xf
+	v_fmac_f32_dpp v138, v139, v19 row_ror:9 row_mask:0xf bank_mask:0xf
+	v_fmac_f32_dpp v1, v139, v4 row_ror:2 row_mask:0xf bank_mask:0xf
+	v_fmac_f32_dpp v138, v139, v20 row_ror:10 row_mask:0xf bank_mask:0xf
+	v_fmac_f32_dpp v1, v139, v5 row_ror:3 row_mask:0xf bank_mask:0xf
+	v_fmac_f32_dpp v138, v139, v21 row_ror:11 row_mask:0xf bank_mask:0xf
+	v_fmac_f32_dpp v1, v139, v10 row_ror:4 row_mask:0xf bank_mask:0xf
+	v_fmac_f32_dpp v138, v139, v22 row_ror:12 row_mask:0xf bank_mask:0xf
+	v_fmac_f32_dpp v1, v139, v11 row_ror:5 row_mask:0xf bank_mask:0xf
+	v_fmac_f32_dpp v138, v139, v23 row_ror:13 row_mask:0xf bank_mask:0xf
+	v_fmac_f32_dpp v1, v139, v12 row_ror:6 row_mask:0xf bank_mask:0xf
+	v_fmac_f32_dpp v138, v139, v24 row_ror:14 row_mask:0xf bank_mask:0xf
+	v_fmac_f32_dpp v1, v139, v13 row_ror:7 row_mask:0xf bank_mask:0xf
+	v_fmac_f32_dpp v138, v139, v25 row_ror:15 row_mask:0xf bank_mask:0xf
+	v_add_f32_e32 v139, v1, v138
+	v_add_f32_e32 v140, v1, v138
+	s_nop 1
+	v_permlane32_swap_b32_e32 v139, v140
+	v_mul_f32_e32 v1, 0xbfb8aa3b, v139
+	v_exp_f32_e32 v1, v1
+	v_sub_f32_e32 v138, v141, v140
+	v_mul_f32_e32 v192, v138, v1
+	v_mul_f32_e32 v193, v138, v1
+	v_sub_f32_e32 v189, v189, v139
+	s_nop 0
+	v_permlane16_swap_b32_e32 v192, v193
+	v_pk_mul_f32 v[196:197], s[54:55], v[164:165]
+	v_pk_mul_f32 v[194:195], s[54:55], v[192:193]
+	v_pk_mul_f32 v[202:203], v[196:197], v[196:197] neg_lo:[0,1] neg_hi:[0,1]
+	v_mov_b32_e32 v198, v195
+	v_mov_b32_dpp v199, v194 row_ror:15 row_mask:0xf bank_mask:0xf bound_ctrl:1
+	v_pk_mul_f32 v[200:201], v[194:195], v[194:195] neg_lo:[0,1] neg_hi:[0,1]
+	v_pk_add_f32 v[198:199], v[198:199], v[202:203]
+	v_pk_add_f32 v[200:201], v[196:197], v[200:201]
+	v_pk_mul_f32 v[198:199], v[198:199], v[198:199]
+	v_pk_mul_f32 v[200:201], v[200:201], v[200:201]
+	v_pk_add_f32 v[194:195], v[194:195], 1.0 op_sel_hi:[1,0] neg_lo:[1,0] neg_hi:[1,0]
+	v_pk_add_f32 v[196:197], v[196:197], 1.0 op_sel_hi:[1,0] neg_lo:[1,0] neg_hi:[1,0]
+	v_pk_mul_f32 v[200:201], v[200:201], s[18:19] op_sel_hi:[1,0]
+	v_pk_mul_f32 v[198:199], v[198:199], s[18:19] op_sel_hi:[1,0]
+	v_pk_mul_f32 v[194:195], v[194:195], v[194:195]
+	v_pk_mul_f32 v[196:197], v[196:197], v[196:197]
+	v_pk_add_f32 v[194:195], v[194:195], v[200:201]
+	v_pk_add_f32 v[196:197], v[196:197], v[198:199]
+	v_cndmask_b32_e64 v142, 0, v194, s[2:3]
+	v_cndmask_b32_e64 v185, 0, v196, s[4:5]
+	v_add_f32_e32 v142, v142, v185
+	v_cndmask_b32_e64 v185, 0, v195, s[6:7]
+	v_add_f32_e32 v142, v185, v142
+	v_cndmask_b32_e64 v185, 0, v197, s[8:9]
+	v_add_f32_e32 v142, v185, v142
+	s_nop 1
+	v_add_f32_dpp v189, v189, v189 row_ror:8 row_mask:0xf bank_mask:0xf bound_ctrl:1
+	v_add_f32_dpp v142, v142, v142 row_ror:8 row_mask:0xf bank_mask:0xf bound_ctrl:1
+	s_nop 0
+	v_add_f32_dpp v189, v189, v189 row_ror:4 row_mask:0xf bank_mask:0xf bound_ctrl:1
+	v_add_f32_dpp v142, v142, v142 row_ror:4 row_mask:0xf bank_mask:0xf bound_ctrl:1
+	s_nop 0
+	v_add_f32_dpp v189, v189, v189 row_ror:2 row_mask:0xf bank_mask:0xf bound_ctrl:1
+	v_add_f32_dpp v142, v142, v142 row_ror:2 row_mask:0xf bank_mask:0xf bound_ctrl:1
+	s_nop 0
+	v_add_f32_dpp v185, v189, v189 row_ror:1 row_mask:0xf bank_mask:0xf bound_ctrl:1
+	v_add_f32_dpp v189, v189, v189 row_ror:1 row_mask:0xf bank_mask:0xf bound_ctrl:1
+	v_add_f32_dpp v142, v142, v142 row_ror:1 row_mask:0xf bank_mask:0xf bound_ctrl:1
+	s_nop 0
+	v_permlane16_swap_b32_e32 v189, v185
+	v_add_f32_e32 v189, v189, v185
+	ds_read_b128 v[138:141], v176
+	ds_read_b32 v1, v178
+	ds_read_b32 v190, v179 offset:12352
+	v_cvt_f64_f32_e32 v[194:195], v142
+	v_max3_f32 v142, |v165|, |v164|, |v193|
+	v_max_f32_e64 v164, |v192|, |v192|
+	v_max_f32_e32 v142, v142, v164
+	v_cmp_nlt_f32_e32 vcc, 1.0, v142
+	s_cmp_eq_u64 vcc, -1
+	v_sub_f32_e32 v142, v189, v177
+	s_cselect_b64 s[12:13], -1, 0
+	v_cndmask_b32_e64 v185, v182, v142, s[12:13]
+	v_mul_f32_e32 v164, 0x3fb8aa3b, v185
+	v_exp_f32_e32 v191, v164
+	v_cmp_le_f64_e64 vcc, |v[194:195]|, s[20:21]
+	v_min_f32_e32 v191, 1.0, v191
+	s_nop 0
+	v_cndmask_b32_e64 v165, v180, -v195, vcc
+	v_cndmask_b32_e32 v164, v181, v194, vcc
+	v_cmp_u_f32_e32 vcc, v185, v185
+	v_cmp_lt_f64_e64 s[14:15], s[30:31], v[164:165]
+	s_nop 0
+	v_cndmask_b32_e32 v185, v191, v185, vcc
+	v_cmp_lt_f32_e32 vcc, v168, v185
+	s_and_b64 s[68:69], s[52:53], vcc
+	s_and_b64 vcc, exec, s[10:11]
+	s_and_b64 s[14:15], s[68:69], s[14:15]
+	s_cbranch_vccnz 62
+	v_cvt_f64_f32_e32 v[192:193], v142
+	v_add_f64 v[194:195], v[164:165], -v[144:145]
+	v_add_f64 v[192:193], v[194:195], v[192:193]
+	v_cndmask_b32_e64 v193, v183, v193, s[12:13]
+	v_cndmask_b32_e64 v192, 0, v192, s[12:13]
+	v_mul_f64 v[194:195], v[192:193], s[56:57]
+	v_rndne_f64_e32 v[194:195], v[194:195]
+	v_fma_f64 v[196:197], s[58:59], v[194:195], v[192:193]
+	v_fmac_f64_e32 v[196:197], s[60:61], v[194:195]
+	v_mov_b64_e32 v[198:199], v[146:147]
+	v_fmac_f64_e32 v[198:199], s[62:63], v[196:197]
+	v_mov_b64_e32 v[200:201], v[148:149]
+	v_fmac_f64_e32 v[200:201], v[196:197], v[198:199]
+	v_mov_b64_e32 v[198:199], v[150:151]
+	v_fmac_f64_e32 v[198:199], v[196:197], v[200:201]
+	v_mov_b64_e32 v[200:201], v[152:153]
+	v_fmac_f64_e32 v[200:201], v[196:197], v[198:199]
+	v_mov_b64_e32 v[198:199], v[154:155]
+	v_fmac_f64_e32 v[198:199], v[196:197], v[200:201]
+	v_mov_b64_e32 v[200:201], v[156:157]
+	v_fmac_f64_e32 v[200:201], v[196:197], v[198:199]
+	v_mov_b64_e32 v[198:199], v[158:159]
+	v_fmac_f64_e32 v[198:199], v[196:197], v[200:201]
+	v_mov_b64_e32 v[200:201], v[160:161]
+	v_fmac_f64_e32 v[200:201], v[196:197], v[198:199]
+	v_mov_b64_e32 v[198:199], v[162:163]
+	v_fmac_f64_e32 v[198:199], v[196:197], v[200:201]
+	v_fma_f64 v[198:199], v[196:197], v[198:199], 1.0
+	v_fma_f64 v[196:197], v[196:197], v[198:199], 1.0
+	v_cvt_i32_f64_e32 v142, v[194:195]
+	v_ldexp_f64 v[194:195], v[196:197], v142
+	v_min_f64 v[194:195], v[194:195], 1.0
+	v_cmp_nlt_f64_e32 vcc, s[64:65], v[192:193]
+	v_cmp_ngt_f64_e64 s[12:13], s[66:67], v[192:193]
+	s_andn2_b64 s[14:15], s[14:15], exec
+	v_cndmask_b32_e32 v142, v184, v195, vcc
+	s_and_b64 vcc, s[12:13], vcc
+	v_cndmask_b32_e64 v193, 0, v142, s[12:13]
+	v_cndmask_b32_e32 v192, 0, v194, vcc
+	v_cvt_f64_f32_e32 v[194:195], v168
+	v_cmp_gt_f64_e32 vcc, v[192:193], v[194:195]
+	s_and_b64 s[12:13], s[52:53], vcc
+	s_and_b64 s[12:13], s[12:13], exec
+	s_or_b64 s[14:15], s[14:15], s[12:13]
+	v_mov_b32_e32 v142, v173
+	v_cndmask_b32_e64 v185, 0, 1, s[14:15]
+	s_and_saveexec_b64 s[12:13], s[16:17]
+	s_cbranch_execnz 6
+	s_branch 8
+	v_cndmask_b32_e64 v142, 0, 1, s[68:69]
+	v_cndmask_b32_e64 v185, 0, 1, s[14:15]
+	s_and_saveexec_b64 s[12:13], s[16:17]
+	v_mov_b32_e32 v168, s51
+	ds_write_b32 v168, v185
+	s_or_b64 exec, exec, s[12:13]
+	v_cndmask_b32_e64 v29, v29, v187, s[14:15]
+	v_cndmask_b32_e64 v93, v93, v188, s[14:15]
+	v_cndmask_b32_e64 v143, v143, v186, s[14:15]
+	v_cndmask_b32_e64 v89, v89, v169, s[14:15]
+	v_cndmask_b32_e64 v177, v177, v189, s[14:15]
+	s_waitcnt lgkmcnt(0)
+	v_fma_f32 v188, v138, v190, v29
+	v_fma_f32 v187, v139, v190, v143
+	v_fma_f32 v189, v140, v190, v93
+	v_fma_f32 v186, v141, v190, v89
+	v_cndmask_b32_e64 v144, v144, v164, s[14:15]
+	s_waitcnt lgkmcnt(0)
+	s_barrier
+	v_cndmask_b32_e64 v145, v145, v165, s[14:15]
+	v_mov_b32_e32 v138, v187
+	v_mov_b32_e32 v139, v186
+	v_bfi_b32 v164, v171, v189, v188
+	v_mov_b32_dpp v138, v187 row_ror:8 row_mask:0xa bank_mask:0xf
+	v_mov_b32_dpp v139, v186 row_ror:8 row_mask:0xa bank_mask:0xf
+	v_fma_f32 v140, v138, v94, v90
+	v_mul_f32_e32 v141, v139, v102
+	v_fmac_f32_dpp v141, v139, v103 row_ror:1 row_mask:0xf bank_mask:0xf
+	v_fmac_f32_dpp v140, v138, v95 row_ror:1 row_mask:0xf bank_mask:0xf
+	v_fmac_f32_dpp v141, v139, v104 row_ror:2 row_mask:0xf bank_mask:0xf
+	v_fmac_f32_dpp v140, v138, v96 row_ror:2 row_mask:0xf bank_mask:0xf
+	v_fmac_f32_dpp v141, v139, v105 row_ror:3 row_mask:0xf bank_mask:0xf
+	v_fmac_f32_dpp v140, v138, v97 row_ror:3 row_mask:0xf bank_mask:0xf
+	v_fmac_f32_dpp v141, v139, v106 row_ror:4 row_mask:0xf bank_mask:0xf
+	v_fmac_f32_dpp v140, v138, v98 row_ror:4 row_mask:0xf bank_mask:0xf
+	v_fmac_f32_dpp v141, v139, v107 row_ror:5 row_mask:0xf bank_mask:0xf
+	v_fmac_f32_dpp v140, v138, v99 row_ror:5 row_mask:0xf bank_mask:0xf
+	v_fmac_f32_dpp v141, v139, v108 row_ror:6 row_mask:0xf bank_mask:0xf
+	v_fmac_f32_dpp v140, v138, v100 row_ror:6 row_mask:0xf bank_mask:0xf
+	v_fmac_f32_dpp v141, v139, v109 row_ror:7 row_mask:0xf bank_mask:0xf
+	v_fmac_f32_dpp v140, v138, v101 row_ror:7 row_mask:0xf bank_mask:0xf
+	v_add_f32_e32 v139, v140, v141
+	v_mov_b32_dpp v138, v141 row_ror:8 row_mask:0xf bank_mask:0xf
+	v_add_f32_dpp v138, v140, v138 row_ror:8 row_mask:0xf bank_mask:0xf
+	s_nop 1
+	v_permlane16_swap_b32_e32 v139, v138
+	v_add_f32_e32 v140, v139, v138
+	v_exp_f32_e32 v138, v140
+	v_max_f32_e32 v139, 0, v140
+	v_add_f32_e32 v138, 1.0, v138
+	v_rcp_f32_e32 v138, v138
+	s_nop 0
+	v_fma_f32 v138, v138, -2.0, 1.0
+	v_bfi_b32 v140, v170, v139, v138
+	v_fma_f32 v138, v140, v110, v91
+	s_nop 0
+	v_mul_f32_dpp v139, v140, v111 row_ror:1 row_mask:0xf bank_mask:0xf
+	v_fmac_f32_dpp v138, v140, v112 row_ror:2 row_mask:0xf bank_mask:0xf
+	v_fmac_f32_dpp v139, v140, v113 row_ror:3 row_mask:0xf bank_mask:0xf
+	v_fmac_f32_dpp v138, v140, v114 row_ror:4 row_mask:0xf bank_mask:0xf
+	v_fmac_f32_dpp v139, v140, v115 row_ror:5 row_mask:0xf bank_mask:0xf
+	v_fmac_f32_dpp v138, v140, v116 row_ror:6 row_mask:0xf bank_mask:0xf
+	v_fmac_f32_dpp v139, v140, v117 row_ror:7 row_mask:0xf bank_mask:0xf
+	v_add_f32_e32 v140, v138, v139
+	v_add_f32_e32 v141, v138, v139
+	s_nop 1
+	v_permlane16_swap_b32_e32 v140, v141
+	v_add_f32_e32 v140, v140, v141
+	v_exp_f32_e32 v138, v140
+	v_max_f32_e32 v139, 0, v140
+	v_add_f32_e32 v138, 1.0, v138
+	v_rcp_f32_e32 v138, v138
+	s_nop 0
+	v_fma_f32 v138, v138, -2.0, 1.0
+	v_bfi_b32 v140, v170, v139, v138
+	v_fma_f32 v138, v140, v118, v92
+	v_mov_b32_e32 v139, 0
+	v_fmac_f32_dpp v139, v140, v122 row_ror:8 row_mask:0xf bank_mask:0xf
+	v_fmac_f32_dpp v138, v140, v119 row_ror:1 row_mask:0xf bank_mask:0xf
+	v_fmac_f32_dpp v139, v140, v123 row_ror:9 row_mask:0xf bank_mask:0xf
+	v_fmac_f32_dpp v138, v140, v120 row_ror:2 row_mask:0xf bank_mask:0xf
+	v_fmac_f32_dpp v139, v140, v124 row_ror:10 row_mask:0xf bank_mask:0xf
+	v_fmac_f32_dpp v138, v140, v121 row_ror:3 row_mask:0xf bank_mask:0xf
+	v_fmac_f32_dpp v139, v140, v125 row_ror:11 row_mask:0xf bank_mask:0xf
+	v_fmac_f32_dpp v138, v140, v126 row_ror:4 row_mask:0xf bank_mask:0xf
+	v_fmac_f32_dpp v139, v140, v130 row_ror:12 row_mask:0xf bank_mask:0xf
+	v_fmac_f32_dpp v138, v140, v127 row_ror:5 row_mask:0xf bank_mask:0xf
+	v_fmac_f32_dpp v139, v140, v131 row_ror:13 row_mask:0xf bank_mask:0xf
+	v_fmac_f32_dpp v138, v140, v128 row_ror:6 row_mask:0xf bank_mask:0xf
+	v_fmac_f32_dpp v139, v140, v132 row_ror:14 row_mask:0xf bank_mask:0xf
+	v_fmac_f32_dpp v138, v140, v129 row_ror:7 row_mask:0xf bank_mask:0xf
+	v_fmac_f32_dpp v139, v140, v133 row_ror:15 row_mask:0xf bank_mask:0xf
+	v_add_f32_e32 v140, v138, v139
+	v_add_f32_e32 v141, v138, v139
+	s_nop 1
+	v_permlane32_swap_b32_e32 v140, v141
+	v_mul_f32_e32 v138, 0xbfb8aa3b, v140
+	v_exp_f32_e32 v138, v138
+	v_sub_f32_e32 v139, v164, v141
+	v_mul_f32_e32 v168, v139, v138
+	v_mul_f32_e32 v169, v139, v138
+	v_mul_f32_e32 v190, -1.0, v140
+	s_nop 0
+	v_permlane16_swap_b32_e32 v168, v169
+	s_nop 0
+	v_mov_b32_e32 v138, v168
+	v_mov_b32_e32 v139, v169
+	v_bfi_b32 v191, v171, v186, v187
+	v_mov_b32_dpp v138, v168 row_ror:8 row_mask:0xa bank_mask:0xf
+	v_mov_b32_dpp v139, v169 row_ror:8 row_mask:0xa bank_mask:0xf
+	v_fma_f32 v140, v138, v50, v86
+	v_mul_f32_e32 v141, v139, v34
+	v_fmac_f32_dpp v141, v139, v35 row_ror:1 row_mask:0xf bank_mask:0xf
+	v_fmac_f32_dpp v140, v138, v51 row_ror:1 row_mask:0xf bank_mask:0xf
+	v_fmac_f32_dpp v141, v139, v36 row_ror:2 row_mask:0xf bank_mask:0xf
+	v_fmac_f32_dpp v140, v138, v52 row_ror:2 row_mask:0xf bank_mask:0xf
+	v_fmac_f32_dpp v141, v139, v37 row_ror:3 row_mask:0xf bank_mask:0xf
+	v_fmac_f32_dpp v140, v138, v53 row_ror:3 row_mask:0xf bank_mask:0xf
+	v_fmac_f32_dpp v141, v139, v58 row_ror:4 row_mask:0xf bank_mask:0xf
+	v_fmac_f32_dpp v140, v138, v54 row_ror:4 row_mask:0xf bank_mask:0xf
+	v_fmac_f32_dpp v141, v139, v59 row_ror:5 row_mask:0xf bank_mask:0xf
+	v_fmac_f32_dpp v140, v138, v55 row_ror:5 row_mask:0xf bank_mask:0xf
+	v_fmac_f32_dpp v141, v139, v60 row_ror:6 row_mask:0xf bank_mask:0xf
+	v_fmac_f32_dpp v140, v138, v56 row_ror:6 row_mask:0xf bank_mask:0xf
+	v_fmac_f32_dpp v141, v139, v61 row_ror:7 row_mask:0xf bank_mask:0xf
+	v_fmac_f32_dpp v140, v138, v57 row_ror:7 row_mask:0xf bank_mask:0xf
+	v_add_f32_e32 v139, v140, v141
+	v_mov_b32_dpp v138, v141 row_ror:8 row_mask:0xf bank_mask:0xf
+	v_add_f32_dpp v138, v140, v138 row_ror:8 row_mask:0xf bank_mask:0xf
+	s_nop 1
+	v_permlane16_swap_b32_e32 v139, v138
+	v_add_f32_e32 v140, v139, v138
+	v_exp_f32_e32 v138, v140
+	v_max_f32_e32 v139, 0, v140
+	v_add_f32_e32 v138, 1.0, v138
+	v_rcp_f32_e32 v138, v138
+	s_nop 0
+	v_fma_f32 v138, v138, -2.0, 1.0
+	v_bfi_b32 v140, v170, v139, v138
+	v_fma_f32 v138, v140, v62, v87
+	s_nop 0
+	v_mul_f32_dpp v139, v140, v63 row_ror:1 row_mask:0xf bank_mask:0xf
+	v_fmac_f32_dpp v138, v140, v64 row_ror:2 row_mask:0xf bank_mask:0xf
+	v_fmac_f32_dpp v139, v140, v65 row_ror:3 row_mask:0xf bank_mask:0xf
+	v_fmac_f32_dpp v138, v140, v66 row_ror:4 row_mask:0xf bank_mask:0xf
+	v_fmac_f32_dpp v139, v140, v67 row_ror:5 row_mask:0xf bank_mask:0xf
+	v_fmac_f32_dpp v138, v140, v68 row_ror:6 row_mask:0xf bank_mask:0xf
+	v_fmac_f32_dpp v139, v140, v69 row_ror:7 row_mask:0xf bank_mask:0xf
+	v_add_f32_e32 v140, v138, v139
+	v_add_f32_e32 v141, v138, v139
+	s_nop 1
+	v_permlane16_swap_b32_e32 v140, v141
+	v_add_f32_e32 v140, v140, v141
+	v_exp_f32_e32 v138, v140
+	v_max_f32_e32 v139, 0, v140
+	v_add_f32_e32 v138, 1.0, v138
+	v_rcp_f32_e32 v138, v138
+	s_nop 0
+	v_fma_f32 v138, v138, -2.0, 1.0
+	v_bfi_b32 v140, v170, v139, v138
+	v_fma_f32 v138, v140, v70, v88
+	v_mov_b32_e32 v139, 0
+	v_fmac_f32_dpp v139, v140, v78 row_ror:8 row_mask:0xf bank_mask:0xf
+	v_fmac_f32_dpp v138, v140, v71 row_ror:1 row_mask:0xf bank_mask:0xf
+	v_fmac_f32_dpp v139, v140, v79 row_ror:9 row_mask:0xf bank_mask:0xf
+	v_fmac_f32_dpp v138, v140, v72 row_ror:2 row_mask:0xf bank_mask:0xf
+	v_fmac_f32_dpp v139, v140, v80 row_ror:10 row_mask:0xf bank_mask:0xf
+	v_fmac_f32_dpp v138, v140, v73 row_ror:3 row_mask:0xf bank_mask:0xf
+	v_fmac_f32_dpp v139, v140, v81 row_ror:11 row_mask:0xf bank_mask:0xf
+	v_fmac_f32_dpp v138, v140, v74 row_ror:4 row_mask:0xf bank_mask:0xf
+	v_fmac_f32_dpp v139, v140, v82 row_ror:12 row_mask:0xf bank_mask:0xf
+	v_fmac_f32_dpp v138, v140, v75 row_ror:5 row_mask:0xf bank_mask:0xf
+	v_fmac_f32_dpp v139, v140, v83 row_ror:13 row_mask:0xf bank_mask:0xf
+	v_fmac_f32_dpp v138, v140, v76 row_ror:6 row_mask:0xf bank_mask:0xf
+	v_fmac_f32_dpp v139, v140, v84 row_ror:14 row_mask:0xf bank_mask:0xf
+	v_fmac_f32_dpp v138, v140, v77 row_ror:7 row_mask:0xf bank_mask:0xf
+	v_fmac_f32_dpp v139, v140, v85 row_ror:15 row_mask:0xf bank_mask:0xf
+	v_add_f32_e32 v140, v138, v139
+	v_add_f32_e32 v141, v138, v139
+	s_nop 1
+	v_permlane32_swap_b32_e32 v140, v141
+	v_mul_f32_e32 v138, 0xbfb8aa3b, v140
+	v_exp_f32_e32 v138, v138
+	v_sub_f32_e32 v139, v191, v141
+	v_mul_f32_e32 v164, v139, v138
+	v_mul_f32_e32 v165, v139, v138
+	v_sub_f32_e32 v190, v190, v140
+	s_nop 0
+	v_permlane16_swap_b32_e32 v164, v165
+	s_nop 0
+	v_mov_b32_e32 v138, v164
+	v_mov_b32_e32 v139, v165
+	v_bfi_b32 v191, v171, v169, v168
+	v_mov_b32_dpp v138, v164 row_ror:8 row_mask:0xa bank_mask:0xf
+	v_mov_b32_dpp v139, v165 row_ror:8 row_mask:0xa bank_mask:0xf
+	v_fma_f32 v140, v138, v30, v26
+	v_mul_f32_e32 v141, v139, v42
+	v_fmac_f32_dpp v141, v139, v43 row_ror:1 row_mask:0xf bank_mask:0xf
+	v_fmac_f32_dpp v140, v138, v31 row_ror:1 row_mask:0xf bank_mask:0xf
+	v_fmac_f32_dpp v141, v139, v44 row_ror:2 row_mask:0xf bank_mask:0xf
+	v_fmac_f32_dpp v140, v138, v32 row_ror:2 row_mask:0xf bank_mask:0xf
+	v_fmac_f32_dpp v141, v139, v45 row_ror:3 row_mask:0xf bank_mask:0xf
+	v_fmac_f32_dpp v140, v138, v33 row_ror:3 row_mask:0xf bank_mask:0xf
+	v_fmac_f32_dpp v141, v139, v46 row_ror:4 row_mask:0xf bank_mask:0xf
+	v_fmac_f32_dpp v140, v138, v38 row_ror:4 row_mask:0xf bank_mask:0xf
+	v_fmac_f32_dpp v141, v139, v47 row_ror:5 row_mask:0xf bank_mask:0xf
+	v_fmac_f32_dpp v140, v138, v39 row_ror:5 row_mask:0xf bank_mask:0xf
+	v_fmac_f32_dpp v141, v139, v48 row_ror:6 row_mask:0xf bank_mask:0xf
+	v_fmac_f32_dpp v140, v138, v40 row_ror:6 row_mask:0xf bank_mask:0xf
+	v_fmac_f32_dpp v141, v139, v49 row_ror:7 row_mask:0xf bank_mask:0xf
+	v_fmac_f32_dpp v140, v138, v41 row_ror:7 row_mask:0xf bank_mask:0xf
+	v_add_f32_e32 v139, v140, v141
+	v_mov_b32_dpp v138, v141 row_ror:8 row_mask:0xf bank_mask:0xf
+	v_add_f32_dpp v138, v140, v138 row_ror:8 row_mask:0xf bank_mask:0xf
+	s_nop 1
+	v_permlane16_swap_b32_e32 v139, v138
+	v_add_f32_e32 v140, v139, v138
+	v_exp_f32_e32 v138, v140
+	v_max_f32_e32 v139, 0, v140
+	v_add_f32_e32 v138, 1.0, v138
+	v_rcp_f32_e32 v138, v138
+	s_nop 0
+	v_fma_f32 v138, v138, -2.0, 1.0
+	v_bfi_b32 v140, v170, v139, v138
+	v_fma_f32 v138, v140, v6, v27
+	s_nop 0
+	v_mul_f32_dpp v139, v140, v7 row_ror:1 row_mask:0xf bank_mask:0xf
+	v_fmac_f32_dpp v138, v140, v8 row_ror:2 row_mask:0xf bank_mask:0xf
+	v_fmac_f32_dpp v139, v140, v9 row_ror:3 row_mask:0xf bank_mask:0xf
+	v_fmac_f32_dpp v138, v140, v14 row_ror:4 row_mask:0xf bank_mask:0xf
+	v_fmac_f32_dpp v139, v140, v15 row_ror:5 row_mask:0xf bank_mask:0xf
+	v_fmac_f32_dpp v138, v140, v16 row_ror:6 row_mask:0xf bank_mask:0xf
+	v_fmac_f32_dpp v139, v140, v17 row_ror:7 row_mask:0xf bank_mask:0xf
+	v_add_f32_e32 v140, v138, v139
+	v_add_f32_e32 v141, v138, v139
+	s_nop 1
+	v_permlane16_swap_b32_e32 v140, v141
+	v_add_f32_e32 v140, v140, v141
+	v_exp_f32_e32 v138, v140
+	v_max_f32_e32 v139, 0, v140
+	v_add_f32_e32 v138, 1.0, v138
+	v_rcp_f32_e32 v138, v138
+	s_nop 0
+	v_fma_f32 v138, v138, -2.0, 1.0
+	v_bfi_b32 v140, v170, v139, v138
+	v_fma_f32 v138, v140, v2, v28
+	v_mov_b32_e32 v139, 0
+	v_fmac_f32_dpp v139, v140, v18 row_ror:8 row_mask:0xf bank_mask:0xf
+	v_fmac_f32_dpp v138, v140, v3 row_ror:1 row_mask:0xf bank_mask:0xf
+	v_fmac_f32_dpp v139, v140, v19 row_ror:9 row_mask:0xf bank_mask:0xf
+	v_fmac_f32_dpp v138, v140, v4 row_ror:2 row_mask:0xf bank_mask:0xf
+	v_fmac_f32_dpp v139, v140, v20 row_ror:10 row_mask:0xf bank_mask:0xf
+	v_fmac_f32_dpp v138, v140, v5 row_ror:3 row_mask:0xf bank_mask:0xf
+	v_fmac_f32_dpp v139, v140, v21 row_ror:11 row_mask:0xf bank_mask:0xf
+	v_fmac_f32_dpp v138, v140, v10 row_ror:4 row_mask:0xf bank_mask:0xf
+	v_fmac_f32_dpp v139, v140, v22 row_ror:12 row_mask:0xf bank_mask:0xf
+	v_fmac_f32_dpp v138, v140, v11 row_ror:5 row_mask:0xf bank_mask:0xf
+	v_fmac_f32_dpp v139, v140, v23 row_ror:13 row_mask:0xf bank_mask:0xf
+	v_fmac_f32_dpp v138, v140, v12 row_ror:6 row_mask:0xf bank_mask:0xf
+	v_fmac_f32_dpp v139, v140, v24 row_ror:14 row_mask:0xf bank_mask:0xf
+	v_fmac_f32_dpp v138, v140, v13 row_ror:7 row_mask:0xf bank_mask:0xf
+	v_fmac_f32_dpp v139, v140, v25 row_ror:15 row_mask:0xf bank_mask:0xf
+	v_add_f32_e32 v140, v138, v139
+	v_add_f32_e32 v141, v138, v139
+	s_nop 1
+	v_permlane32_swap_b32_e32 v140, v141
+	v_mul_f32_e32 v138, 0xbfb8aa3b, v140
+	v_exp_f32_e32 v138, v138
+	v_sub_f32_e32 v139, v191, v141
+	v_mul_f32_e32 v192, v139, v138
+	v_mul_f32_e32 v193, v139, v138
+	v_sub_f32_e32 v190, v190, v140
+	s_nop 0
+	v_permlane16_swap_b32_e32 v192, v193
+	v_pk_mul_f32 v[196:197], s[54:55], v[164:165]
+	v_pk_mul_f32 v[194:195], s[54:55], v[192:193]
+	v_pk_mul_f32 v[202:203], v[196:197], v[196:197] neg_lo:[0,1] neg_hi:[0,1]
+	v_mov_b32_e32 v198, v195
+	v_mov_b32_dpp v199, v194 row_ror:15 row_mask:0xf bank_mask:0xf bound_ctrl:1
+	v_pk_mul_f32 v[200:201], v[194:195], v[194:195] neg_lo:[0,1] neg_hi:[0,1]
+	v_pk_add_f32 v[198:199], v[198:199], v[202:203]
+	v_pk_add_f32 v[200:201], v[196:197], v[200:201]
+	v_pk_mul_f32 v[198:199], v[198:199], v[198:199]
+	v_pk_mul_f32 v[200:201], v[200:201], v[200:201]
+	v_pk_add_f32 v[194:195], v[194:195], 1.0 op_sel_hi:[1,0] neg_lo:[1,0] neg_hi:[1,0]
+	v_pk_add_f32 v[196:197], v[196:197], 1.0 op_sel_hi:[1,0] neg_lo:[1,0] neg_hi:[1,0]
+	v_pk_mul_f32 v[200:201], v[200:201], s[18:19] op_sel_hi:[1,0]
+	v_pk_mul_f32 v[198:199], v[198:199], s[18:19] op_sel_hi:[1,0]
+	v_pk_mul_f32 v[194:195], v[194:195], v[194:195]
+	v_pk_mul_f32 v[196:197], v[196:197], v[196:197]
+	v_pk_add_f32 v[194:195], v[194:195], v[200:201]
+	v_pk_add_f32 v[196:197], v[196:197], v[198:199]
+	v_cndmask_b32_e64 v191, 0, v194, s[2:3]
+	v_cndmask_b32_e64 v194, 0, v196, s[4:5]
+	v_add_f32_e32 v191, v191, v194
+	v_cndmask_b32_e64 v194, 0, v195, s[6:7]
+	v_max3_f32 v164, |v165|, |v164|, |v193|
+	v_max_f32_e64 v165, |v192|, |v192|
+	v_add_f32_e32 v191, v194, v191
+	v_cndmask_b32_e64 v194, 0, v197, s[8:9]
+	v_max_f32_e32 v164, v164, v165
+	v_add_f32_e32 v191, v194, v191
+	v_cmp_nlt_f32_e32 vcc, 1.0, v164
+	s_nop 1
+	v_add_f32_dpp v190, v190, v190 row_ror:8 row_mask:0xf bank_mask:0xf bound_ctrl:1
+	v_add_f32_dpp v191, v191, v191 row_ror:8 row_mask:0xf bank_mask:0xf bound_ctrl:1
+	s_nop 0
+	v_add_f32_dpp v190, v190, v190 row_ror:4 row_mask:0xf bank_mask:0xf bound_ctrl:1
+	v_add_f32_dpp v191, v191, v191 row_ror:4 row_mask:0xf bank_mask:0xf bound_ctrl:1
+	s_nop 0
+	v_add_f32_dpp v190, v190, v190 row_ror:2 row_mask:0xf bank_mask:0xf bound_ctrl:1
+	v_add_f32_dpp v191, v191, v191 row_ror:2 row_mask:0xf bank_mask:0xf bound_ctrl:1
+	s_nop 0
+	v_add_f32_dpp v194, v190, v190 row_ror:1 row_mask:0xf bank_mask:0xf bound_ctrl:1
+	v_add_f32_dpp v190, v190, v190 row_ror:1 row_mask:0xf bank_mask:0xf bound_ctrl:1
+	v_add_f32_dpp v191, v191, v191 row_ror:1 row_mask:0xf bank_mask:0xf bound_ctrl:1
+	s_nop 0
+	v_permlane16_swap_b32_e32 v190, v194
+	v_add_f32_e32 v190, v190, v194
+	s_cmp_eq_u64 vcc, -1
+	v_cvt_f64_f32_e32 v[194:195], v191
+	v_sub_f32_e32 v191, v190, v177
+	s_cselect_b64 s[12:13], -1, 0
+	v_cndmask_b32_e64 v192, v182, v191, s[12:13]
+	v_mul_f32_e32 v164, 0x3fb8aa3b, v192
+	v_exp_f32_e32 v193, v164
+	v_mov_b32_e32 v168, s85
+	ds_read_b128 v[138:141], v176 offset:1024
+	ds_read_b32 v168, v168 offset:16
+	ds_read_b32 v169, v179 offset:12356
+	v_cmp_le_f64_e64 vcc, |v[194:195]|, s[20:21]
+	v_min_f32_e32 v193, 1.0, v193
+	s_nop 0
+	v_cndmask_b32_e64 v165, v180, -v195, vcc
+	v_cndmask_b32_e32 v164, v181, v194, vcc
+	v_cmp_u_f32_e32 vcc, v192, v192
+	v_cmp_lt_f64_e64 s[14:15], s[30:31], v[164:165]
+	s_nop 0
+	v_cndmask_b32_e32 v192, v193, v192, vcc
+	v_cmp_lt_f32_e32 vcc, v1, v192
+	s_and_b64 s[68:69], s[52:53], vcc
+	s_and_b64 vcc, exec, s[10:11]
+	s_and_b64 s[14:15], s[68:69], s[14:15]
+	s_cbranch_vccnz 62
+	v_cvt_f64_f32_e32 v[192:193], v191
+	v_add_f64 v[194:195], v[164:165], -v[144:145]
+	v_add_f64 v[192:193], v[194:195], v[192:193]
+	v_cndmask_b32_e64 v193, v183, v193, s[12:13]
+	v_cndmask_b32_e64 v192, 0, v192, s[12:13]
+	v_mul_f64 v[194:195], v[192:193], s[56:57]
+	v_rndne_f64_e32 v[194:195], v[194:195]
+	v_fma_f64 v[196:197], s[58:59], v[194:195], v[192:193]
+	v_fmac_f64_e32 v[196:197], s[60:61], v[194:195]
+	v_mov_b64_e32 v[198:199], v[146:147]
+	v_fmac_f64_e32 v[198:199], s[62:63], v[196:197]
+	v_mov_b64_e32 v[200:201], v[148:149]
+	v_fmac_f64_e32 v[200:201], v[196:197], v[198:199]
+	v_mov_b64_e32 v[198:199], v[150:151]
+	v_fmac_f64_e32 v[198:199], v[196:197], v[200:201]
+	v_mov_b64_e32 v[200:201], v[152:153]
+	v_fmac_f64_e32 v[200:201], v[196:197], v[198:199]
+	v_mov_b64_e32 v[198:199], v[154:155]
+	v_fmac_f64_e32 v[198:199], v[196:197], v[200:201]
+	v_mov_b64_e32 v[200:201], v[156:157]
+	v_fmac_f64_e32 v[200:201], v[196:197], v[198:199]
+	v_mov_b64_e32 v[198:199], v[158:159]
+	v_fmac_f64_e32 v[198:199], v[196:197], v[200:201]
+	v_mov_b64_e32 v[200:201], v[160:161]
+	v_fmac_f64_e32 v[200:201], v[196:197], v[198:199]
+	v_mov_b64_e32 v[198:199], v[162:163]
+	v_fmac_f64_e32 v[198:199], v[196:197], v[200:201]
+	v_fma_f64 v[198:199], v[196:197], v[198:199], 1.0
+	v_fma_f64 v[196:197], v[196:197], v[198:199], 1.0
+	v_cvt_i32_f64_e32 v191, v[194:195]
+	v_ldexp_f64 v[194:195], v[196:197], v191
+	v_min_f64 v[194:195], v[194:195], 1.0
+	v_cmp_nlt_f64_e32 vcc, s[64:65], v[192:193]
+	v_cmp_ngt_f64_e64 s[12:13], s[66:67], v[192:193]
+	s_andn2_b64 s[14:15], s[14:15], exec
+	v_cndmask_b32_e32 v191, v184, v195, vcc
+	s_and_b64 vcc, s[12:13], vcc
+	v_cndmask_b32_e64 v193, 0, v191, s[12:13]
+	v_cndmask_b32_e32 v192, 0, v194, vcc
+	v_cvt_f64_f32_e32 v[194:195], v1
+	v_cmp_gt_f64_e32 vcc, v[192:193], v[194:195]
+	s_and_b64 s[12:13], s[52:53], vcc
+	s_and_b64 s[12:13], s[12:13], exec
+	s_or_b64 s[14:15], s[14:15], s[12:13]
+	v_mov_b32_e32 v1, v173
+	v_cndmask_b32_e64 v191, 0, 1, s[14:15]
+	s_and_saveexec_b64 s[12:13], s[16:17]
+	s_cbranch_execz 64320
+	s_branch 64316
```

Result: slower. 1.036 billion (-1.5%).
